# beast-dev/beast-mcmc

Measured on NVIDIA H100. Metric: tree log-likelihood evals/sec, higher is better.
Workload: dtype f64

## Files before the change

beast-mcmc_b200/csrc/api.cu:

```cuda
#include "../../include/libhmsbeagle_b200.h"
#include "engine.h"
#include "multi.h"

#include <algorithm>
#include <atomic>
#include <chrono>
#include <cmath>
#include <cstdio>
#include <cstdlib>
#include <cstring>
#include <string>
#include <unordered_map>

using namespace b200;

namespace {

std::mutex gMutex;
std::vector<Instance*> gInstances;

const long kSupportedFlags =
    BEAGLE_FLAG_PRECISION_DOUBLE | BEAGLE_FLAG_PRECISION_SINGLE | BEAGLE_FLAG_COMPUTATION_SYNCH | BEAGLE_FLAG_EIGEN_REAL |
    BEAGLE_FLAG_EIGEN_COMPLEX | BEAGLE_FLAG_SCALING_MANUAL | BEAGLE_FLAG_SCALING_DYNAMIC |
    BEAGLE_FLAG_SCALERS_RAW | BEAGLE_FLAG_SCALERS_LOG | BEAGLE_FLAG_VECTOR_NONE | BEAGLE_FLAG_THREADING_NONE |
// ... 58 lines not shown
            cudaEventCreate(&a);
            cudaEventCreate(&b);
            cudaEventRecord(a, in->stream);
        }
    }
    ~TimedScope() {
        if (in->timing) {
            cudaEventRecord(b, in->stream);
            in->timed[cls].push_back({a, b});
        }
    }
};

void* stage(Instance* in, const void* src, size_t bytes) {
    size_t need = (bytes + 255) & ~size_t(255);
    if (need > in->stageSize) return nullptr;
    if (in->stagePos + need > in->stageSize) {
        cudaStreamSynchronize(in->stream);
        in->stagePos = 0;
    }
    char* h = in->hStage + in->stagePos;
    char* d = in->dStage + in->stagePos;
    memcpy(h, src, bytes);
    if (cudaMemcpyAsync(d, h, bytes, cudaMemcpyHostToDevice, in->stream) != cudaSuccess) return nullptr;
    in->stagePos += need;
    return d;
}

int uploadSmall(Instance* in, void* dDst, const void* src, size_t bytes) {
    size_t need = (bytes + 255) & ~size_t(255);
    if (need > in->stageSize) return BEAGLE_ERROR_OUT_OF_RANGE;
    if (in->stagePos + need > in->stageSize) {
        cudaStreamSynchronize(in->stream);
        in->stagePos = 0;
    }
    char* h = in->hStage + in->stagePos;
    memcpy(h, src, bytes);
    in->stagePos += need;
    CUDA_OK(cudaMemcpyAsync(dDst, h, bytes, cudaMemcpyHostToDevice, in->stream));
    return BEAGLE_SUCCESS;
}

char* ensurePartials(Instance* in, int idx) {
    if (in->partials[idx] == nullptr) {
        if (in->nextSlot >= in->nSlots) return nullptr;
        in->slotOf[idx] = in->nextSlot++;
        in->partials[idx] = in->partialsBase + (size_t)in->slotOf[idx] * in->partialsElems * in->elemBytes();
    }
    return in->partials[idx];
}

bool validRange(int idx, int n) { return idx >= 0 && idx < n; }

void destroyInstance(Instance* in) {
    if (in->shard != nullptr) { shardedDestroy(in); delete in; return; }
    cudaSetDevice(in->device);
    exchangeRelease(in);
    if (in->stream) cudaStreamSynchronize(in->stream);
    cudaFree(in->partialsBase); cudaFree(in->states8Base); cudaFree(in->states32Base);
    for (CachedPlan& cp : in->planCache) { cp.dropGraph(); cudaFree(cp.dBlock); }
    cudaFree(in->dEigen); cudaFree(in->dMat); cudaFree(in->dEvec); cudaFree(in->dIncSums); cudaFree(in->dIncCounter);
    cudaFree(in->dRecipe);
    if (in->hMapped) cudaFreeHost(in->hMapped); cudaFree(in->dRates); cudaFree(in->dWeights);
    cudaFree(in->dFreqs); cudaFree(in->dScale); cudaFree(in->dPatternWeights);
    cudaFree(in->dPatternPartitions); cudaFree(in->dSite); cudaFree(in->dBlockSums); cudaFree(in->dOut);
    cudaFree(in->dCounter); cudaFree(in->dStage); cudaFree(in->dScratch);
    if (in->hStage) cudaFreeHost(in->hStage);
    if (in->hOut) cudaFreeHost(in->hOut);
    for (int c = 0; c < T_CLASSES; ++c)
        for (auto& ev : in->timed[c]) { cudaEventDestroy(ev.first); cudaEventDestroy(ev.second); }
    if (in->stream) cudaStreamDestroy(in->stream);
    delete in;
}

std::vector<BeagleResource> gResources;
std::vector<int> gShardDevices;
int gShardResource = -1;
std::vector<std::string> gResourceStrings;
BeagleResourceList gResourceList = {nullptr, 0};
std::once_flag gResourceOnce;

void buildResources() {
    int n = 0;
    if (cudaGetDeviceCount(&n) != cudaSuccess) { cudaGetLastError(); n = 0; }
    gResourceStrings.reserve(2 * (n + 1));
    gResourceStrings.push_back("CPU (host)");
    gResourceStrings.push_back("no host implementation in this library | use a GPU resource (1..N)");
    for (int d = 0; d < n; ++d) {
        cudaDeviceProp prop;
        if (cudaGetDeviceProperties(&prop, d) != cudaSuccess) { cudaGetLastError(); continue; }
        char buf[512];
        snprintf(buf, sizeof buf, "%s", prop.name);
        gResourceStrings.push_back(buf);
        snprintf(buf, sizeof buf, "Global memory (MB): %zu | SMs: %d | compute capability: %d.%d | "
                 "native walk kernels (sm_90a), fp64 arithmetic, fp64 or fp32 (4-state) partials",
                 (size_t)(prop.totalGlobalMem >> 20), prop.multiProcessorCount, prop.major, prop.minor);
        gResourceStrings.push_back(buf);
    }
    gShardDevices.clear();
    if (const char* env = getenv("B200_SHARD_DEVICES")) {
        for (const char* q = env; *q;) {
            char* end = nullptr;
            const long d = strtol(q, &end, 10);
            if (end == q) break;
            if (d >= 0 && d < n) gShardDevices.push_back((int)d);
            q = (*end == ',') ? end + 1 : end;
        }
    } else {
        for (int d = 0; d < n; ++d) gShardDevices.push_back(d);
    }
    if (gShardDevices.size() > (size_t)kMaxGroup) gShardDevices.resize(kMaxGroup);
    if (!gShardDevices.empty()) {
        char buf[512];
        snprintf(buf, sizeof buf, "GPU x %zu (pattern-sharded)", gShardDevices.size());
        gResourceStrings.push_back(buf);
        snprintf(buf, sizeof buf, "one instance over %zu GPUs | contiguous pattern blocks (Patterns.java:142-169 rule) | "
                 "per-shard sums added over NVLink inside the root kernel", gShardDevices.size());
        gResourceStrings.push_back(buf);
        gShardResource = (int)(gResourceStrings.size() / 2) - 1;
    }
    size_t count = gResourceStrings.size() / 2;
    gResources.resize(count);
    for (size_t r = 0; r < count; ++r) {
        gResources[r].name = const_cast<char*>(gResourceStrings[2 * r].c_str());
        gResources[r].description = const_cast<char*>(gResourceStrings[2 * r + 1].c_str());
        gResources[r].supportFlags = (r == 0) ? (BEAGLE_FLAG_PROCESSOR_CPU | BEAGLE_FLAG_FRAMEWORK_CPU) : kSupportedFlags;
        gResources[r].requiredFlags = (r == 0) ? BEAGLE_FLAG_FRAMEWORK_CPU : BEAGLE_FLAG_FRAMEWORK_CUDA;
    }
    gResourceList.list = gResources.data();
    gResourceList.length = (int)count;
}

char gImplName[] = "B200-CUDA-Double";
char gImplNameSingle[] = "B200-CUDA-Single";
char gImplDesc[] = "sm_90a walk kernels: one launch per operation list, shared-memory operand stack";


struct Sub { int begin, end, pBase, pLimit; };
struct Plan {
    std::vector<int> order;
    std::vector<Sub> subs;
    std::vector<int> phaseStart;
};

void planPhases(const std::vector<HostOp>& ops, int nBuffers, bool allowReorder, int fixedT, int wantSubs, int minT,
                int smallRemainder, Plan& plan) {
    const int n = (int)ops.size();
    auto single = [&]() {
        plan.order.resize(n);
        for (int k = 0; k < n; ++k) plan.order[k] = k;
        plan.subs.assign(1, Sub{0, n, 0, 0});
        plan.phaseStart = {0, 1};
    };
    if (!allowReorder || n < 2) { single(); return; }
    std::vector<int> writer(nBuffers, -1);
    for (int k = 0; k < n; ++k) {
        if (writer[ops[k].dest] >= 0) { single(); return; }
        writer[ops[k].dest] = k;
    }
    std::vector<int> ch0(n, -1), ch1(n, -1), parent(n, -1);
    for (int k = 0; k < n; ++k) {
        const int a = writer[ops[k].c1], b = writer[ops[k].c2];
        if (a >= 0) { if (a >= k || parent[a] >= 0) { single(); return; } ch0[k] = a; parent[a] = k; }
        if (b >= 0 && ops[k].c2 != ops[k].c1) { if (b >= k || parent[b] >= 0) { single(); return; } ch1[k] = b; parent[b] = k; }
        if (ops[k].dest == ops[k].c1 || ops[k].dest == ops[k].c2) { single(); return; }
    }
    std::vector<char> alive(n, 1);
    std::vector<int> size(n), need(n);
    std::vector<std::pair<int, int>> stack;
    plan.order.clear(); plan.order.reserve(n);
    plan.subs.clear(); plan.phaseStart.assign(1, 0);
    int remaining = n;
    while (remaining > 0) {
        const int T = fixedT > 0 ? fixedT : (remaining <= smallRemainder ? remaining : std::max(minT, (remaining + wantSubs - 1) / wantSubs));
        for (int k = 0; k < n; ++k) {
            if (!alive[k]) continue;
            const int a = (ch0[k] >= 0 && alive[ch0[k]]) ? ch0[k] : -1;
            const int b = (ch1[k] >= 0 && alive[ch1[k]]) ? ch1[k] : -1;
            size[k] = 1 + (a >= 0 ? size[a] : 0) + (b >= 0 ? size[b] : 0);
            int na = a >= 0 ? need[a] : 0, nb = b >= 0 ? need[b] : 0;
            if (na < nb) std::swap(na, nb);
            need[k] = std::max(1, std::max(na, nb + (nb > 0 ? 1 : 0)));
        }
        for (int r = 0; r < n; ++r) {
            if (!alive[r] || size[r] > T) continue;
            if (parent[r] >= 0 && size[parent[r]] <= T) continue;
            const int begin = (int)plan.order.size();
            stack.push_back({r, 0});
            while (!stack.empty()) {
                auto [k, stageNo] = stack.back();
                stack.pop_back();
                if (stageNo == 1) { plan.order.push_back(k); continue; }
                stack.push_back({k, 1});
                const int a = (ch0[k] >= 0 && alive[ch0[k]]) ? ch0[k] : -1;
                const int b = (ch1[k] >= 0 && alive[ch1[k]]) ? ch1[k] : -1;
                const int na = a >= 0 ? need[a] : -1, nb = b >= 0 ? need[b] : -1;
                if (na >= nb) { if (b >= 0) stack.push_back({b, 0}); if (a >= 0) stack.push_back({a, 0}); }
                else          { if (a >= 0) stack.push_back({a, 0}); if (b >= 0) stack.push_back({b, 0}); }
            }
            plan.subs.push_back(Sub{begin, (int)plan.order.size(), 0, 0});
        }
        for (int q = plan.subs[plan.phaseStart.back()].begin; q < (int)plan.order.size(); ++q) alive[plan.order[q]] = 0;
        std::stable_sort(plan.subs.begin() + plan.phaseStart.back(), plan.subs.end(),
                         [](const Sub& a, const Sub& b) { return (a.end - a.begin) > (b.end - b.begin); });
        remaining = n - (int)plan.order.size();
        plan.phaseStart.push_back((int)plan.subs.size());
    }
}

void planLevels(const std::vector<HostOp>& ops, int nBuffers, Plan& plan) {
    const int n = (int)ops.size();
    std::vector<int> writer(nBuffers, -1), level(n, 0);
    bool hazard = false;
    for (int k = 0; k < n; ++k) { if (writer[ops[k].dest] >= 0) hazard = true; writer[ops[k].dest] = k; }
    int maxLevel = 0;
    for (int k = 0; k < n && !hazard; ++k) {
        for (int src : {ops[k].c1, ops[k].c2}) {
            const int w = writer[src];
            if (w < 0) continue;
            if (w >= k) { hazard = true; break; }
            level[k] = std::max(level[k], level[w] + 1);
        }
        maxLevel = std::max(maxLevel, level[k]);
    }
    plan.order.resize(n);
    for (int k = 0; k < n; ++k) plan.order[k] = k;
    plan.subs.clear();
    if (hazard) { plan.subs.assign(1, Sub{0, n, 0, 0}); plan.phaseStart = {0, 1}; return; }
    std::stable_sort(plan.order.begin(), plan.order.end(), [&](int a, int b) { return level[a] < level[b]; });
    plan.phaseStart.assign(1, 0);
    for (int pos = 0; pos < n; ++pos) {
        if (pos > 0 && level[plan.order[pos]] != level[plan.order[pos - 1]]) plan.phaseStart.push_back((int)plan.subs.size());
        plan.subs.push_back(Sub{pos, pos + 1, 0, 0});
    }
    plan.phaseStart.push_back((int)plan.subs.size());
}

void planPreorderPhases(const std::vector<HostOp>& ops, int nBuffers, int fixedT, int wantSubs, int minT,
                        int smallRemainder, Plan& plan) {
    const int n = (int)ops.size();
    std::vector<int> writer(nBuffers, -1), parent(n, -1);
    bool ok = n >= 2;
    for (int k = 0; k < n && ok; ++k) { ok = writer[ops[k].dest] < 0; writer[ops[k].dest] = k; }
    for (int k = 0; k < n && ok; ++k) {
        const int a = writer[ops[k].c1];
        ok = writer[ops[k].c2] < 0 && (a < 0 || a < k) && ops[k].dest != ops[k].c1 && ops[k].dest != ops[k].c2;
        parent[k] = a;
    }
    if (!ok) { planLevels(ops, nBuffers, plan); return; }
    std::vector<std::vector<int>> kids(n);
    for (int k = 0; k < n; ++k) if (parent[k] >= 0) kids[parent[k]].push_back(k);
    std::vector<char> alive(n, 1);
    std::vector<int> size(n), stack;
    std::vector<std::vector<int>> phases;
    int remaining = n;
    while (remaining > 0) {
        const int T = fixedT > 0 ? fixedT : (remaining <= smallRemainder ? remaining : std::max(minT, (remaining + wantSubs - 1) / wantSubs));
        for (int k = n - 1; k >= 0; --k) {
            if (!alive[k]) continue;
            size[k] = 1;
            for (int c : kids[k]) if (alive[c]) size[k] += size[c];
        }
        std::vector<int> roots;
        for (int r = 0; r < n; ++r)
            if (alive[r] && size[r] <= T && !(parent[r] >= 0 && alive[parent[r]] && size[parent[r]] <= T)) roots.push_back(r);
        for (int r : roots) {
            stack.assign(1, r);
            while (!stack.empty()) {
                const int k = stack.back(); stack.pop_back();
                if (!alive[k]) continue;
                alive[k] = 0; --remaining;
                for (int c : kids[k]) if (alive[c]) stack.push_back(c);
            }
        }
        phases.push_back(std::move(roots));
    }
    std::vector<int> phaseOf(n, -1), rootOf(n, -1);
    for (int ph = 0; ph < (int)phases.size(); ++ph)
        for (int r : phases[ph]) { phaseOf[r] = ph; rootOf[r] = r; }
    for (int k = 0; k < n; ++k)
        if (rootOf[k] < 0) { rootOf[k] = rootOf[parent[k]]; phaseOf[k] = phaseOf[parent[k]]; }
    plan.order.clear(); plan.order.reserve(n);
    plan.subs.clear(); plan.phaseStart.assign(1, 0);
    for (int ph = (int)phases.size() - 1; ph >= 0; --ph) {
        for (int r : phases[ph]) {
            const int begin = (int)plan.order.size();
            stack.assign(1, r);
            while (!stack.empty()) {
                const int k = stack.back(); stack.pop_back();
                plan.order.push_back(k);
                for (int q = (int)kids[k].size() - 1; q >= 0; --q)
                    if (rootOf[kids[k][q]] == r) stack.push_back(kids[k][q]);
            }
            plan.subs.push_back(Sub{begin, (int)plan.order.size(), 0, 0});
        }
        std::stable_sort(plan.subs.begin() + plan.phaseStart.back(), plan.subs.end(),
                         [](const Sub& a, const Sub& b) { return (a.end - a.begin) > (b.end - b.begin); });
        plan.phaseStart.push_back((int)plan.subs.size());
    }
}

cudaError_t launchPlan(Instance* in, const void* dOps, const void* dSubs, const std::vector<int>& phaseStart,
                       const std::vector<int>& phaseDepth, bool fourPath, int maxWindow, bool preOrder, int eigenSlot = -1,
                       bool aligned = false, const void* dSnap = nullptr, int nSnap = 0, const void* dVirtTips = nullptr) {
    const bool virt = dVirtTips != nullptr;
    cudaError_t e = cudaSuccess;
    if (nSnap > 0) {
        TimedScope ts(in, T_PARTIALS);
        e = launchCherrySnapshot(in, static_cast<const int4*>(dSnap), nSnap);
    }
    for (size_t ph = 0; ph + 1 < phaseStart.size() && e == cudaSuccess; ++ph) {
        const int s0 = phaseStart[ph], s1 = phaseStart[ph + 1];
        if (s1 <= s0) continue;
        TimedScope ts(in, T_PARTIALS);
        if (fourPath && eigenSlot >= 0 && !preOrder && (ph >= phaseDepth.size() || phaseDepth[ph] == 0)) {
            e = launchWalk4E(in, static_cast<const Op4*>(dOps), static_cast<const int4*>(dSubs) + s0, s1 - s0, maxWindow,
                             aligned, in->hEigen.data() + (size_t)eigenSlot * 36, static_cast<const int4*>(dVirtTips));
            continue;
        }
        if (virt) return cudaErrorInvalidValue;
        e = fourPath ? launchWalk4(in, static_cast<const Op4*>(dOps), static_cast<const int4*>(dSubs) + s0, s1 - s0,
                                   ph < phaseDepth.size() ? phaseDepth[ph] : 0, maxWindow, preOrder)
                     : launchWalkGeneric(in, static_cast<const DevOp*>(dOps), static_cast<const int4*>(dSubs) + s0, s1 - s0,
                                         maxWindow, preOrder);
    }
    return e;
}

cudaError_t accumulateInList(Instance* in, const std::vector<CumGroup>& groups) {
    for (const CumGroup& g : groups) {
        int* dIdx = static_cast<int*>(stage(in, g.indices.data(), sizeof(int) * g.indices.size()));
        if (dIdx == nullptr) return cudaErrorMemoryAllocation;
        cudaError_t e = launchScaleAccumulate(in, dIdx, (int)g.indices.size(), in->dScale + (size_t)g.cum * in->Ppad, 1.0,
                                              g.pBegin, g.pEnd);
        if (e != cudaSuccess) return e;
        in->scaleIsLog[g.cum] = 1;
    }
    return cudaSuccess;
}

void noteScaleWrites(Instance* in, const std::vector<HostOp>& hops) {
    for (const HostOp& o : hops) if (o.sw >= 0) in->scaleIsLog[o.sw] = in->logScalers ? 1 : 0;
}


cudaError_t storeCherries(Instance* in, const int* bufs, int count) {
    if (in->cherryTip1.empty()) return cudaSuccess;
    std::vector<int4> items;
    for (int k = 0; k < count; ++k) {
        const int b = bufs[k];
        if (!validRange(b, in->nBuffers) || in->cherryTip1[b] < 0 || in->cherryStored[b]) continue;
        items.push_back(make_int4(in->slotOf[b], b, in->cherryTip1[b], in->cherryTip2[b]));
        in->cherryStored[b] = 1;
    }
    if (items.empty()) return cudaSuccess;
    const int4* dItems = static_cast<const int4*>(stage(in, items.data(), sizeof(int4) * items.size()));
    cudaError_t e = cudaErrorMemoryAllocation;
    if (dItems != nullptr) {
        TimedScope ts(in, T_PARTIALS);
        e = launchCherryStore(in, dItems, (int)items.size());
    }
    if (e != cudaSuccess) for (const int4& it : items) in->cherryStored[it.y] = 0;
    return e;
}

cudaError_t storeExternal(Instance* in, const std::vector<CherryRef>& external) {
    std::vector<int> bufs;
    for (const CherryRef& x : external) if (x.tip1 < 0) bufs.push_back(x.buf);
    return storeCherries(in, bufs.data(), (int)bufs.size());
}

cudaError_t settleCherriesOf(Instance* in, int t) {
    std::vector<int> deps;
    for (int b = 0; b < (int)in->cherryTip1.size(); ++b)
        if (in->cherryTip1[b] >= 0 && (in->cherryTip1[b] == t || in->cherryTip2[b] == t)) deps.push_back(b);
    const cudaError_t e = storeCherries(in, deps.data(), (int)deps.size());
    if (e == cudaSuccess) for (int b : deps) in->cherryTip1[b] = -1;
    return e;
}

void noteCherryWrites(Instance* in, const std::vector<HostOp>& hops, const std::vector<CherryRef>& cherries) {
    if (in->cherryTip1.empty()) return;
    for (const HostOp& o : hops) in->cherryTip1[o.dest] = -1;
    for (const CherryRef& c : cherries) {
        in->cherryTip1[c.buf] = c.tip1; in->cherryTip2[c.buf] = c.tip2; in->cherryStored[c.buf] = 0;
    }
}

int prepareOps(Instance* in, const std::vector<HostOp>& hops, bool byPartition) {
    for (const HostOp& o : hops) {
        if (!validRange(o.dest, in->nBuffers) || !validRange(o.c1, in->nBuffers) ||
            !validRange(o.c2, in->nBuffers) || !validRange(o.m1, in->nMatrices) ||
            !validRange(o.m2, in->nMatrices))
            return BEAGLE_ERROR_OUT_OF_RANGE;
        if (o.sw != BEAGLE_OP_NONE && !validRange(o.sw, in->nScale)) return BEAGLE_ERROR_OUT_OF_RANGE;
        if (o.sr != BEAGLE_OP_NONE && !validRange(o.sr, in->nScale)) return BEAGLE_ERROR_OUT_OF_RANGE;
        if (o.cum != BEAGLE_OP_NONE && !validRange(o.cum, in->nScale)) return BEAGLE_ERROR_OUT_OF_RANGE;
        if (byPartition && !validRange(o.part, in->partitionCount)) return BEAGLE_ERROR_OUT_OF_RANGE;
    }
    {
        std::vector<char> written(in->nBuffers, 0);
        for (const HostOp& o : hops) written[o.dest] = 1;
        auto holdsData = [&](int b) { return written[b] || in->partials[b] != nullptr || in->states32[b] != nullptr; };
        for (const HostOp& o : hops) {
            if (!holdsData(o.c1) || !holdsData(o.c2)) return BEAGLE_ERROR_OUT_OF_RANGE;
            if (o.kind == 1 && !written[o.c1] && in->states32[o.c1] != nullptr) return BEAGLE_ERROR_OUT_OF_RANGE;
        }
    }
    for (const HostOp& o : hops) {
        if (ensurePartials(in, o.dest) == nullptr) return BEAGLE_ERROR_OUT_OF_MEMORY;
        if (in->states32[o.dest] != nullptr) in->bufferEpoch++;
        in->states8[o.dest] = nullptr;
        in->states32[o.dest] = nullptr;
    }
    return BEAGLE_SUCCESS;
}

int eigenFormSlot(const Instance* in, const std::vector<HostOp>& hops) {
    if (!in->eigenWalk || in->matCP == 0 || in->walkVariant != 0 || hops.empty() || hops[0].kind == 1) return -1;
    const int E = in->matEigen[hops[0].m1];
    if (E < 0 || !in->eigenReal[E]) return -1;
    const unsigned gen = in->eigenGen[E];
    for (const HostOp& o : hops)
        if (in->matEigen[o.m1] != E || in->matEigen[o.m2] != E || in->matEigenGen[o.m1] != gen || in->matEigenGen[o.m2] != gen)
            return -1;
    return E;
}

int planAndLaunch(Instance* in, const std::vector<HostOp>& hops, bool byPartition) {
    const int n = (int)hops.size();
    if (n == 0) return BEAGLE_SUCCESS;
    static_assert(sizeof(HostOp) == 10 * sizeof(int), "HostOp is compared bytewise");
    if (in->planCacheSize > 0) {
        for (CachedPlan& cp : in->planCache) {
            if (cp.dBlock == nullptr || cp.n != n || cp.byPartition != byPartition || cp.epoch != in->bufferEpoch ||
                memcmp(cp.key.data(), hops.data(), sizeof(HostOp) * (size_t)n) != 0)
                continue;
            const int eigenSlot = cp.fourPath ? eigenFormSlot(in, hops) : -1;
            bool stale = cp.readsVirtual && eigenSlot < 0;
            for (const CherryRef& x : cp.external)
                stale = stale || (x.tip1 >= 0 && (in->cherryTip1[x.buf] != x.tip1 || in->cherryTip2[x.buf] != x.tip2));
            if (stale) { cp.dropGraph(); cp.n = -1; continue; }
            CUDA_OK(storeExternal(in, cp.external));
            cp.lastUse = ++in->planClock;
            cp.hits++;
            const unsigned eigenGenNow = eigenSlot >= 0 ? in->eigenGen[eigenSlot] : 0u;
            const void* dSnap = static_cast<char*>(cp.dBlock) + cp.snapOffset;
            const int nSnap = (int)cp.cherries.size();
            const void* dTips = cp.readsVirtual ? static_cast<char*>(cp.dBlock) + cp.tipsOffset : nullptr;
            if (cp.graphExec != nullptr && (cp.graphEigen != eigenSlot || cp.graphEigenGen != eigenGenNow)) {
                if (cp.graphAllEigen && eigenSlot >= 0 && cp.graphEigen == eigenSlot &&
                    updateWalk4EGraph(cp.graphExec, cp.graphKernelNodes, in->hEigen.data() + (size_t)eigenSlot * 36) == cudaSuccess) {
                    cp.graphEigenGen = eigenGenNow;
                } else {
                    cudaGetLastError();
                    cp.dropGraph();
                    cp.hits = 1;
                    if (++cp.graphInvalidations >= 4) cp.graphFailed = true;
                }
            }
            int launches = nSnap > 0;
            for (size_t ph = 0; ph + 1 < cp.phaseStart.size(); ++ph) launches += cp.phaseStart[ph + 1] > cp.phaseStart[ph];
            if (in->useGraphs && launches >= 2 && cp.cumGroups.empty()) {
                if (cp.graphExec == nullptr && !cp.graphFailed && cp.hits >= 2 && !in->timing &&
                    cudaStreamBeginCapture(in->stream, cudaStreamCaptureModeThreadLocal) == cudaSuccess) {
                    const cudaError_t e1 = launchPlan(in, cp.dBlock, static_cast<char*>(cp.dBlock) + cp.subsOffset, cp.phaseStart,
                                                      cp.phaseDepth, cp.fourPath, cp.maxWindow, cp.preOrder, eigenSlot,
                                                      !cp.byPartition, dSnap, nSnap, dTips);
                    cp.graphEigen = eigenSlot;
                    cp.graphEigenGen = eigenGenNow;
                    cudaGraph_t g = nullptr;
                    const cudaError_t e2 = cudaStreamEndCapture(in->stream, &g);
                    if (e1 != cudaSuccess || e2 != cudaSuccess || g == nullptr ||
                        cudaGraphInstantiate(&cp.graphExec, g, 0) != cudaSuccess) {
                        cp.graphExec = nullptr;
                        cp.graphFailed = true;
                        if (g) cudaGraphDestroy(g);
                    } else {
                        cp.graph = g;
                        cp.graphKernelNodes.clear();
                        cp.graphAllEigen = cp.fourPath && eigenSlot >= 0 && !cp.preOrder;
                        for (int dpt : cp.phaseDepth) cp.graphAllEigen = cp.graphAllEigen && dpt == 0;
                        size_t nn = 0;
                        if (cudaGraphGetNodes(g, nullptr, &nn) == cudaSuccess && nn > 0) {
                            std::vector<cudaGraphNode_t> nodes(nn);
                            cudaGraphNodeType ty;
                            if (cudaGraphGetNodes(g, nodes.data(), &nn) == cudaSuccess)
                                for (size_t q = 0; q < nn; ++q)
                                    if (cudaGraphNodeGetType(nodes[q], &ty) == cudaSuccess && ty == cudaGraphNodeTypeKernel)
                                        cp.graphKernelNodes.push_back(nodes[q]);
                        }
                        if (cp.graphKernelNodes.empty()) cp.graphAllEigen = false;
                    }
                    if (getenv("B200_BEAGLE_DEBUG"))
                        fprintf(stderr, "[b200-beagle] graph %s: %d launches\n", cp.graphExec ? "captured" : "capture failed",
                                launches);
                    cudaGetLastError();
                }
                if (cp.graphExec != nullptr) {
                    TimedScope ts(in, T_PARTIALS, launches);
                    CUDA_OK(cudaGraphLaunch(cp.graphExec, in->stream));
                    noteScaleWrites(in, hops);
                    noteCherryWrites(in, hops, cp.cherries);
                    return BEAGLE_SUCCESS;
                }
            }
            CUDA_OK(launchPlan(in, cp.dBlock, static_cast<char*>(cp.dBlock) + cp.subsOffset, cp.phaseStart, cp.phaseDepth,
                               cp.fourPath, cp.maxWindow, cp.preOrder, eigenSlot, !cp.byPartition, dSnap, nSnap,
                               dTips));
            CUDA_OK(accumulateInList(in, cp.cumGroups));
            noteScaleWrites(in, hops);
            noteCherryWrites(in, hops, cp.cherries);
            return BEAGLE_SUCCESS;
        }
    }
    {
        const int rcPrepare = prepareOps(in, hops, byPartition);
        if (rcPrepare != BEAGLE_SUCCESS) return rcPrepare;
    }
    const bool fourState = in->matCP > 0;
    const bool preOrder = hops[0].kind == 1;
    const int eigenSlot = fourState ? eigenFormSlot(in, hops) : -1;
    std::vector<char> written(in->nBuffers, 0);
    std::vector<int> firstWrite(in->nBuffers, n);
    for (int k = n - 1; k >= 0; --k) { written[hops[k].dest] = 1; firstWrite[hops[k].dest] = k; }
    std::vector<CherryRef> cherries;
    std::vector<int4> snap;
    std::vector<HostOp> kept;
    bool readsVirtual = false;
    if (!in->cherryTip1.empty() && !byPartition && !preOrder && eigenSlot >= 0 && !in->stackTail) {
        std::vector<int> writes(in->nBuffers, 0), firstRead(in->nBuffers, n);
        for (int k = 0; k < n; ++k) {
            writes[hops[k].dest]++;
            firstRead[hops[k].c1] = std::min(firstRead[hops[k].c1], k);
            firstRead[hops[k].c2] = std::min(firstRead[hops[k].c2], k);
        }
        for (int k = 0; k < n; ++k) {
            const HostOp& o = hops[k];
            if (in->states8[o.c1] != nullptr && in->states8[o.c2] != nullptr && o.sw == BEAGLE_OP_NONE &&
                o.sr == BEAGLE_OP_NONE && o.cum == BEAGLE_OP_NONE && writes[o.dest] == 1 && firstRead[o.dest] > k) {
                cherries.push_back(CherryRef{o.dest, o.c1, o.c2});
                snap.push_back(make_int4(o.dest, o.m1, o.m2, 0));
            } else {
                kept.push_back(o);
            }
        }
        if (kept.empty()) { cherries.clear(); snap.clear(); }
        readsVirtual = !cherries.empty();
        for (const HostOp& o : hops)
            for (int c : {o.c1, o.c2})
                readsVirtual = readsVirtual || (!written[c] && in->states32[c] == nullptr && in->cherryTip1[c] >= 0);
    }
    Plan plan;
    int maxWindow = in->Ppad;
    const int patsPerWarp = !fourState ? 16 : (in->walkVariant == 2 ? 8 * in->tensorR : (32 / in->matCP) * in->walkR);
    const int warpsPerSM = fourState ? 32 : 12;
    auto wantSubsFor = [&](int window) {
        const int warpsPerSub = std::max(1, (window + patsPerWarp - 1) / patsPerWarp);
        const int over = in->phaseOversub > 0 ? in->phaseOversub : (warpsPerSub >= 32 ? 1 : 2);
        return std::max(1, over * ((in->smCount * warpsPerSM + warpsPerSub - 1) / warpsPerSub));
    };
    if (!byPartition && !preOrder) {
        planPhases(cherries.empty() ? hops : kept, in->nBuffers, in->reorder != 0, in->phaseT, wantSubsFor(in->Ppad),
                   in->phaseTmin, in->phaseSmall, plan);
        bool served = true;
        for (size_t ph = 0; readsVirtual && ph + 1 < plan.phaseStart.size(); ++ph) {
            const int nSubs = plan.phaseStart[ph + 1] - plan.phaseStart[ph];
            served = served && (nSubs == 0 || walk4pServes(in, nSubs, in->Ppad));
        }
        if (!served) {
            readsVirtual = false;
            if (!cherries.empty()) {
                cherries.clear(); snap.clear(); kept.clear();
                planPhases(hops, in->nBuffers, in->reorder != 0, in->phaseT, wantSubsFor(in->Ppad), in->phaseTmin,
                           in->phaseSmall, plan);
            }
        }
        for (Sub& sb : plan.subs) { sb.pBase = 0; sb.pLimit = in->Ppad; }
    }
    const std::vector<HostOp>& L = cherries.empty() ? hops : kept;
    const int nL = (int)L.size();
    std::vector<int> vt1(readsVirtual ? in->nBuffers : 0, -1), vt2(readsVirtual ? in->nBuffers : 0, -1);
    for (const CherryRef& c : cherries) { vt1[c.buf] = c.tip1; vt2[c.buf] = c.tip2; }
    std::vector<CherryRef> external;
    {
        std::vector<char> seen(in->nBuffers, 0);
        for (int k = 0; k < n; ++k)
            for (int c : {hops[k].c1, hops[k].c2}) {
                if (firstWrite[c] < k || in->states32[c] != nullptr || seen[c]) continue;
                seen[c] = 1;
                const bool virt = readsVirtual && !written[c] && in->cherryTip1[c] >= 0;
                external.push_back(CherryRef{c, virt ? in->cherryTip1[c] : -1, virt ? in->cherryTip2[c] : -1});
                if (virt) { vt1[c] = in->cherryTip1[c]; vt2[c] = in->cherryTip2[c]; }
            }
    }
    CUDA_OK(storeExternal(in, external));
    {
        if (!byPartition) {
            if (preOrder) {
                if (in->prePhases) planPreorderPhases(hops, in->nBuffers, in->phaseT, wantSubsFor(in->Ppad), in->phaseTmin, in->phaseSmall, plan);
                else planLevels(hops, in->nBuffers, plan);
                for (Sub& sb : plan.subs) { sb.pBase = 0; sb.pLimit = in->Ppad; }
            }
        } else {
            std::vector<std::vector<int>> members(in->partitionCount);
            for (int k = 0; k < n; ++k) members[hops[k].part].push_back(k);
            std::vector<Plan> plans;
            std::vector<int> base;
            maxWindow = 1;
            for (int part = 0; part < in->partitionCount; ++part) {
                if (members[part].empty()) continue;
                std::vector<HostOp> sub(members[part].size());
                for (size_t q = 0; q < sub.size(); ++q) sub[q] = hops[members[part][q]];
                Plan pl;
                const int window = in->partEnd[part] - in->partBegin[part];
                if (sub[0].kind == 1 && in->prePhases) planPreorderPhases(sub, in->nBuffers, in->phaseT, wantSubsFor(std::max(1, window)), in->phaseTmin, in->phaseSmall, pl);
                else if (sub[0].kind == 1) planLevels(sub, in->nBuffers, pl);
                else planPhases(sub, in->nBuffers, in->reorder != 0, in->phaseT, wantSubsFor(std::max(1, window)), in->phaseTmin, in->phaseSmall, pl);
                base.push_back((int)plan.order.size());
                for (int idx : pl.order) plan.order.push_back(members[part][idx]);
                for (Sub& sb : pl.subs) {
                    sb.begin += base.back(); sb.end += base.back();
                    sb.pBase = in->partBegin[part]; sb.pLimit = in->partEnd[part];
                }
                maxWindow = std::max(maxWindow, window);
                plans.push_back(std::move(pl));
            }
            plan.phaseStart.assign(1, 0);
            for (size_t ph = 0;; ++ph) {
                bool any = false;
                for (const Plan& pl : plans) {
                    if (ph + 1 >= pl.phaseStart.size()) continue;
                    any = true;
                    for (int q = pl.phaseStart[ph]; q < pl.phaseStart[ph + 1]; ++q) plan.subs.push_back(pl.subs[q]);
                }
                if (!any) break;
                plan.phaseStart.push_back((int)plan.subs.size());
            }
        }
    }
    const std::vector<int>& order = plan.order;

    const bool stackEverywhere = fourState && in->walkVariant == 1 && !preOrder;
    const bool stackThin = fourState && in->walkVariant == 0 && in->stackTail && !preOrder;
    const int maxDepth = (stackEverywhere || stackThin) ? in->stackDepthMax : 0;
    const int nPhases = (int)plan.phaseStart.size() - 1;
    std::vector<char> subStack(plan.subs.size(), 0);
    std::vector<int> phaseDepth(std::max(nPhases, 1), 0), phaseOfSub(plan.subs.size(), 0);
    if (maxDepth > 0) {
        const int patsPerWarpS = (32 / in->matCP) * in->walkR;
        for (int ph = 0; ph < nPhases; ++ph) {
            long warps = 0;
            for (int q = plan.phaseStart[ph]; q < plan.phaseStart[ph + 1]; ++q) {
                warps += (plan.subs[q].pLimit - plan.subs[q].pBase + patsPerWarpS - 1) / patsPerWarpS;
                phaseOfSub[q] = ph;
            }
            const bool thin = warps < (long)in->smCount * 8;
            for (int q = plan.phaseStart[ph]; q < plan.phaseStart[ph + 1]; ++q) subStack[q] = stackEverywhere || thin;
        }
    }
    std::vector<int> lastReadOfProd(maxDepth > 0 ? nL : 0, -1);
    std::vector<int> subOfPos(nL, 0);
    for (int sIdx = 0; sIdx < (int)plan.subs.size(); ++sIdx)
        for (int q = plan.subs[sIdx].begin; q < plan.subs[sIdx].end; ++q) subOfPos[q] = sIdx;
    if (maxDepth > 0) {
        std::vector<int> lastRead(in->nBuffers, -1);
        for (size_t sIdx = 0; sIdx < plan.subs.size(); ++sIdx) {
            if (!subStack[sIdx]) continue;
            const Sub& sb = plan.subs[sIdx];
            for (int pos = sb.end - 1; pos >= sb.begin; --pos) {
                const HostOp& o = L[order[pos]];
                lastReadOfProd[pos] = lastRead[o.dest];
                lastRead[o.dest] = -1;
                if (lastRead[o.c1] < 0) lastRead[o.c1] = pos;
                if (lastRead[o.c2] < 0) lastRead[o.c2] = pos;
            }
            for (int pos = sb.begin; pos < sb.end; ++pos) {
                const HostOp& o = L[order[pos]];
                lastRead[o.dest] = lastRead[o.c1] = lastRead[o.c2] = -1;
            }
        }
    }
    std::vector<int> slotOf(maxDepth > 0 ? in->nBuffers : 0, -1), slotFreeAt(maxDepth > 0 ? in->nBuffers : 0, -1);
    std::vector<int> freeSlots;
    int depthUsed = 0, depthThisSub = 0, curSub = -1;

    const bool fourPath = in->matCP > 0;
    std::vector<CumGroup> cumGroups;
    std::vector<DevOp> dops(fourPath ? 0 : nL);
    std::vector<Op4> ops4(fourPath ? nL : 0);
    std::vector<int4> virtTips(readsVirtual ? nL : 0);
    for (int pos = 0; pos < nL; ++pos) {
        const HostOp& o = L[order[pos]];
        const bool t1 = in->states32[o.c1] != nullptr;
        const bool t2 = in->states32[o.c2] != nullptr;
        int srcSlot1 = -1, srcSlot2 = -1, dstSlot = -1;
        if (maxDepth > 0 && subOfPos[pos] != curSub) {
            curSub = subOfPos[pos];
            freeSlots.clear();
            depthThisSub = 0;
        }
        if (maxDepth > 0 && subStack[subOfPos[pos]]) {
            auto take = [&](int buf, bool isTip) -> int {
                if (isTip) return -1;
                const int slot = slotOf[buf];
                if (slot >= 0 && slotFreeAt[buf] == pos) { freeSlots.push_back(slot); slotOf[buf] = -1; }
                return slot;
            };
            srcSlot1 = take(o.c1, t1);
            srcSlot2 = (o.c2 == o.c1) ? srcSlot1 : take(o.c2, t2);
            if (slotOf[o.dest] >= 0) { freeSlots.push_back(slotOf[o.dest]); slotOf[o.dest] = -1; }
            if (lastReadOfProd[pos] > pos) {
                int slot = -1;
                if (!freeSlots.empty()) { slot = freeSlots.back(); freeSlots.pop_back(); }
                else if (depthThisSub < maxDepth) {
                    slot = depthThisSub++;
                    depthUsed = std::max(depthUsed, depthThisSub);
                    phaseDepth[phaseOfSub[subOfPos[pos]]] = std::max(phaseDepth[phaseOfSub[subOfPos[pos]]], depthThisSub);
                }
                if (slot >= 0) { slotOf[o.dest] = slot; slotFreeAt[o.dest] = lastReadOfProd[pos]; dstSlot = slot; }
            }
        }
        const int pBegin = byPartition ? in->partBegin[o.part] : 0;
        const int pEnd = byPartition ? in->partEnd[o.part] : in->P;
        if (o.cum >= 0 && o.sw >= 0) {
            CumGroup* grp = nullptr;
            for (CumGroup& g : cumGroups) if (g.cum == o.cum && g.pBegin == pBegin && g.pEnd == pEnd) { grp = &g; break; }
            if (grp == nullptr) { cumGroups.push_back(CumGroup{o.cum, pBegin, pEnd, {}}); grp = &cumGroups.back(); }
            grp->indices.push_back(o.sw);
        }
        const int cum = -1;
        if (fourPath) {
            Op4& d = ops4[pos];
            const bool v1 = readsVirtual && !t1 && vt1[o.c1] >= 0, v2 = readsVirtual && !t2 && vt1[o.c2] >= 0;
            d.dest = in->slotOf[o.dest];
            d.c1 = t1 ? -(o.c1 + 1) : v1 ? o.c1 : in->slotOf[o.c1];
            d.c2 = t2 ? -(o.c2 + 1) : v2 ? o.c2 : in->slotOf[o.c2];
            d.m1 = o.m1; d.m2 = o.m2; d.sw = o.sw; d.sr = o.sr; d.cum = cum;
            d.pBegin = pBegin; d.pEnd = pEnd;
            d.slots = (unsigned)(srcSlot1 & 0xFF) | ((unsigned)(srcSlot2 & 0xFF) << 8) | ((unsigned)(dstSlot & 0xFF) << 16);
            d.pad_ = o.kind | (v1 ? 4 : 0) | (v2 ? 8 : 0);
            d.pfA = d.pfB = 0; d.pfM1 = d.pfM2 = -1;
            if (readsVirtual)
                virtTips[pos] = make_int4(v1 ? vt1[o.c1] : 0, v1 ? vt2[o.c1] : 0, v2 ? vt1[o.c2] : 0, v2 ? vt2[o.c2] : 0);
            if (in->forward && !(maxDepth > 0 && subStack[subOfPos[pos]]) && pos > plan.subs[subOfPos[pos]].begin) {
                const Op4& pv = ops4[pos - 1];
                if (pv.pBegin == d.pBegin && pv.pEnd == d.pEnd) {
                    if (!t1 && !v1 && d.c1 == pv.dest) d.pad_ |= 2;
                    else if (!preOrder && !t2 && !v2 && d.c2 == pv.dest) {
                        std::swap(d.c1, d.c2); std::swap(d.m1, d.m2);
                        if (readsVirtual) { int4& t = virtTips[pos]; t = make_int4(t.z, t.w, t.x, t.y); }
                        d.pad_ = (d.pad_ & ~12) | (v1 ? 8 : 0) | 2;
                    }
                }
            }
        } else {
            DevOp& d = dops[pos];
            memset(&d, 0, sizeof d);
            d.dest = reinterpret_cast<double*>(in->partials[o.dest]);
            d.c1 = t1 ? nullptr : reinterpret_cast<const double*>(in->partials[o.c1]);
            d.c2 = t2 ? nullptr : reinterpret_cast<const double*>(in->partials[o.c2]);
            d.s1 = t1 ? (const void*)in->states32[o.c1] : nullptr;
            d.s2 = t2 ? (const void*)in->states32[o.c2] : nullptr;
            d.m1 = in->dMat + (size_t)o.m1 * in->matStride;
            d.m2 = in->dMat + (size_t)o.m2 * in->matStride;
            d.scaleWrite = o.sw >= 0 ? in->dScale + (size_t)o.sw * in->Ppad : nullptr;
            d.scaleRead = o.sr >= 0 ? in->dScale + (size_t)o.sr * in->Ppad : nullptr;
            d.cumScale = cum >= 0 ? in->dScale + (size_t)cum * in->Ppad : nullptr;
            d.pBegin = pBegin; d.pEnd = pEnd;
            d.srcSlot1 = d.srcSlot2 = d.dstSlot = -1;
            d.pad_ = o.kind;
            if (in->forward && !preOrder && pos > plan.subs[subOfPos[pos]].begin) {
                const DevOp& pv = dops[pos - 1];
                if (pv.pBegin == d.pBegin && pv.pEnd == d.pEnd) {
                    if (d.c1 != nullptr && d.c1 == pv.dest) d.pad_ |= 2;
                    else if (d.c2 != nullptr && d.c2 == pv.dest) {
                        std::swap(d.c1, d.c2); std::swap(d.s1, d.s2); std::swap(d.m1, d.m2); d.pad_ |= 2;
                    }
                }
            }
        }
    }
    if (fourPath && in->lookahead && (!preOrder || in->lookaheadPre)) {
        std::vector<char> thick(plan.subs.size(), 0);
        const long perSub = (maxWindow + (32 / in->matCP) * in->walkR - 1) / ((32 / in->matCP) * in->walkR);
        for (int ph = 0; ph < nPhases; ++ph) {
            const bool t = (long)(plan.phaseStart[ph + 1] - plan.phaseStart[ph]) * perSub >= (long)in->smCount * 8;
            for (int q = plan.phaseStart[ph]; q < plan.phaseStart[ph + 1]; ++q) thick[q] = t;
        }
        for (size_t sIdx = 0; sIdx < plan.subs.size(); ++sIdx) {
            if ((maxDepth > 0 && subStack[sIdx]) || (!thick[sIdx] && in->lookahead < 2)) continue;
            for (int pos = plan.subs[sIdx].begin; pos + 1 < plan.subs[sIdx].end; ++pos) {
                Op4& d = ops4[pos];
                const Op4& nx = ops4[pos + 1];
                auto enc = [&](int child, bool fromRegisters, bool virt) -> int {
                    if (fromRegisters || virt) return 0;
                    if (child < 0) return ((-child - 1) << 1) | 1;
                    return child == d.dest ? 0 : ((child + 1) << 1);
                };
                d.pfA = enc(nx.c1, (nx.pad_ & 2) != 0, (nx.pad_ & 4) != 0);
                d.pfB = enc(nx.c2, false, (nx.pad_ & 8) != 0);
                if (d.pfA == 0) { d.pfA = d.pfB; d.pfB = 0; }
                d.pfM1 = nx.m1; d.pfM2 = nx.m2;
            }
        }
    }
    if (fourPath && getenv("B200_BEAGLE_DEBUG")) {
        int fwd = 0, internal = 0;
        for (const Op4& d : ops4) { fwd += (d.pad_ & 2) != 0; internal += (d.c1 >= 0) + (d.c2 >= 0); }
        fprintf(stderr, "[b200-beagle] plan: %d ops (%zu virtual cherries), %zu subtrees, %d phases, %d internal children, "
                "%d forwarded in registers\n", nL, cherries.size(), plan.subs.size(), nPhases, internal, fwd);
    }
    const size_t opBytes = (fourPath ? sizeof(Op4) : sizeof(DevOp)) * (size_t)nL;
    const size_t subBytes = sizeof(Sub) * plan.subs.size();
    const size_t snapBytes = sizeof(int4) * snap.size();
    const size_t subsOffset = (opBytes + 255) & ~size_t(255);
    const size_t snapOffset = subsOffset + ((subBytes + 255) & ~size_t(255));
    const size_t tipsBytes = sizeof(int4) * virtTips.size();
    const size_t tipsOffset = snapOffset + ((snapBytes + 255) & ~size_t(255));
    const size_t blockBytes = tipsOffset + tipsBytes;
    std::vector<char> hBlock(blockBytes, 0);
    memcpy(hBlock.data(), fourPath ? (const void*)ops4.data() : (const void*)dops.data(), opBytes);
    memcpy(hBlock.data() + subsOffset, plan.subs.data(), subBytes);
    if (snapBytes) memcpy(hBlock.data() + snapOffset, snap.data(), snapBytes);
    if (tipsBytes) memcpy(hBlock.data() + tipsOffset, virtTips.data(), tipsBytes);
    void* dOps = stage(in, hBlock.data(), blockBytes);
    void* tmp = nullptr;
    if (dOps == nullptr) {
        CUDA_OK(cudaMalloc(&tmp, blockBytes));
        dOps = tmp;
        cudaError_t ce = cudaMemcpyAsync(dOps, hBlock.data(), blockBytes, cudaMemcpyHostToDevice, in->stream);
        if (ce == cudaSuccess) ce = cudaStreamSynchronize(in->stream);
        if (ce != cudaSuccess) { cudaFree(tmp); CUDA_OK(ce); }
    }
    void* dSubs = static_cast<char*>(dOps) + subsOffset;
    std::vector<int> depths(plan.phaseStart.size(), 0);
    for (size_t ph = 0; ph + 1 < plan.phaseStart.size(); ++ph) depths[ph] = (maxDepth > 0 && ph < phaseDepth.size()) ? phaseDepth[ph] : 0;
    cudaError_t e = launchPlan(in, dOps, dSubs, plan.phaseStart, depths, fourPath, maxWindow, preOrder, eigenSlot, !byPartition,
                               static_cast<char*>(dOps) + snapOffset, (int)snap.size(),
                               readsVirtual ? static_cast<char*>(dOps) + tipsOffset : nullptr);
    if (e == cudaSuccess) e = accumulateInList(in, cumGroups);
    noteScaleWrites(in, hops);
    if (e == cudaSuccess) noteCherryWrites(in, hops, cherries);
    if (e == cudaSuccess && tmp == nullptr && in->planCacheSize > 0) {
        if ((int)in->planCache.size() < in->planCacheSize) in->planCache.emplace_back();
        CachedPlan* slot = nullptr;
        for (CachedPlan& cp : in->planCache) {
            if (cp.dBlock == nullptr || cp.n < 0) { slot = &cp; break; }
            if (slot == nullptr || cp.lastUse < slot->lastUse) slot = &cp;
        }
        slot->dropGraph();
        slot->hits = 0;
        slot->graphFailed = false;
        slot->graphInvalidations = 0;
        if (slot->capacity < blockBytes) {
            if (slot->dBlock) cudaFree(slot->dBlock);
            slot->dBlock = nullptr; slot->capacity = 0;
            if (cudaMalloc(&slot->dBlock, blockBytes) == cudaSuccess) slot->capacity = blockBytes; else cudaGetLastError();
        }
        if (slot->dBlock != nullptr &&
            cudaMemcpyAsync(slot->dBlock, dOps, blockBytes, cudaMemcpyDeviceToDevice, in->stream) == cudaSuccess) {
            slot->key = hops; slot->n = n; slot->byPartition = byPartition; slot->epoch = in->bufferEpoch;
            slot->subsOffset = subsOffset; slot->snapOffset = snapOffset; slot->tipsOffset = tipsOffset;
            slot->cherries = cherries; slot->external = external; slot->readsVirtual = readsVirtual;
            slot->phaseStart = plan.phaseStart; slot->phaseDepth = depths;
            slot->fourPath = fourPath; slot->maxWindow = maxWindow; slot->preOrder = preOrder;
            slot->lastUse = ++in->planClock;
            slot->cumGroups = cumGroups;
            slot->graphFailed = !cumGroups.empty();
        } else if (slot->dBlock != nullptr) {
            slot->n = -1;
        }
    }
    if (tmp != nullptr) { cudaStreamSynchronize(in->stream); cudaFree(tmp); }
    CUDA_OK(e);
    return BEAGLE_SUCCESS;
}

}

namespace b200 {
Instance* instanceById(int id) { return getInstance(id); }
}

extern "C" {

#ifndef B200_SOURCE_HASH
#define B200_SOURCE_HASH "unhashed"
#endif
const char* beagleGetVersion(void) { return "4.0.1-b200+" B200_SOURCE_HASH; }
const char* b200GetSourceHash(void) { return B200_SOURCE_HASH; }

const char* beagleGetCitation(void) {
    return "H100-native tree-likelihood engine exposing the BEAGLE API.\n"
           "API after: Ayres et al. (2019) BEAGLE 3. Syst Biol 68:1052-1061.";
}

BeagleResourceList* beagleGetResourceList(void) {
    std::call_once(gResourceOnce, buildResources);
    return &gResourceList;
}

BeagleBenchmarkedResourceList* beagleGetBenchmarkedResourceList(
    int tipCount, int compactBufferCount, int stateCount, int patternCount, int categoryCount, int* resourceList,
    int resourceCount, long preferenceFlags, long requirementFlags, int eigenModelCount, int partitionCount,
    int calculateDerivatives, long benchmarkFlags);

int beagleCreateInstance(int tipCount, int partialsBufferCount, int compactBufferCount, int stateCount,
                         int patternCount, int eigenBufferCount, int matrixBufferCount, int categoryCount,
                         int scaleBufferCount, int* resourceList, int resourceCount, long preferenceFlags,
                         long requirementFlags, BeagleInstanceDetails* returnInfo) {
    if (tipCount < 0 || partialsBufferCount < 0 || compactBufferCount < 0 || stateCount < 2 ||
        patternCount < 1 || eigenBufferCount < 0 || matrixBufferCount < 0 || categoryCount < 1 ||
        scaleBufferCount < 0 || stateCount > 255)
        return BEAGLE_ERROR_OUT_OF_RANGE;
    if (requirementFlags & ~kSupportedFlags) return BEAGLE_ERROR_NO_RESOURCE;
    const bool singleFits = stateCount <= 4 && categoryCount <= 8;
    if (requirementFlags & BEAGLE_FLAG_PRECISION_SINGLE) {
        if (!singleFits || (requirementFlags & BEAGLE_FLAG_PRECISION_DOUBLE)) return BEAGLE_ERROR_NO_RESOURCE;
    }
    const bool single = singleFits && ((requirementFlags & BEAGLE_FLAG_PRECISION_SINGLE) ||
                                       ((preferenceFlags & BEAGLE_FLAG_PRECISION_SINGLE) &&
                                        !((preferenceFlags | requirementFlags) & BEAGLE_FLAG_PRECISION_DOUBLE)));
    BeagleResourceList* rl = beagleGetResourceList();
    int resource = -1;
    if (resourceList == nullptr || resourceCount <= 0) {
        if (rl->length > 1) resource = 1;
    } else {
        for (int k = 0; k < resourceCount; ++k)
            if (resourceList[k] >= 1 && resourceList[k] < rl->length) { resource = resourceList[k]; break; }
    }
    if (resource < 1) return BEAGLE_ERROR_NO_RESOURCE;

    if (resource == gShardResource) {
        Instance* parent = new Instance();
        parent->resource = resource;
        parent->device = gShardDevices[0];
        parent->P = patternCount; parent->S = stateCount; parent->C = categoryCount; parent->tipCount = tipCount;
        const int g = (int)gShardDevices.size();
        const int rc = shardedCreate(parent, g, gShardDevices.data(), tipCount, partialsBufferCount, compactBufferCount,
                                     stateCount, patternCount, eigenBufferCount, matrixBufferCount, categoryCount,
                                     scaleBufferCount, preferenceFlags, requirementFlags, returnInfo);
        if (rc != BEAGLE_SUCCESS) { delete parent; return rc; }
        if (returnInfo != nullptr) {
            returnInfo->resourceNumber = resource;
            returnInfo->resourceName = rl->list[resource].name;
            parent->flags = returnInfo->flags;
        }
        std::lock_guard<std::mutex> lock(gMutex);
        int id = -1;
        for (size_t k = 0; k < gInstances.size(); ++k) if (gInstances[k] == nullptr) { id = (int)k; break; }
        if (id < 0) { gInstances.push_back(nullptr); id = (int)gInstances.size() - 1; }
        gInstances[id] = parent;
        parent->id = id;
        return id;
    }

    Instance* in = new Instance();
    in->device = resource - 1;
    in->resource = resource;
    if (cudaSetDevice(in->device) != cudaSuccess) { delete in; return BEAGLE_ERROR_NO_RESOURCE; }
    in->tipCount = tipCount; in->nPartials = partialsBufferCount; in->nCompact = compactBufferCount;
    in->S = stateCount; in->P = patternCount; in->nEigen = eigenBufferCount; in->nMatrices = matrixBufferCount;
    in->C = categoryCount; in->nScale = scaleBufferCount;
    in->Sp = stateCount <= 4 ? 4 : ((stateCount + 7) / 8) * 8;
    in->Ppad = ((patternCount + 31) / 32) * 32;
    in->nBuffers = partialsBufferCount + compactBufferCount;
    in->nSets = std::max(1, eigenBufferCount);
    in->single = single;
    in->complexEigen = (requirementFlags | preferenceFlags) & BEAGLE_FLAG_EIGEN_COMPLEX;
    in->logScalers = (requirementFlags | preferenceFlags) & BEAGLE_FLAG_SCALERS_LOG;
    in->flags = (single ? BEAGLE_FLAG_PRECISION_SINGLE : BEAGLE_FLAG_PRECISION_DOUBLE) | BEAGLE_FLAG_COMPUTATION_SYNCH |
                BEAGLE_FLAG_SCALING_MANUAL |
                BEAGLE_FLAG_VECTOR_NONE | BEAGLE_FLAG_THREADING_NONE | BEAGLE_FLAG_PROCESSOR_GPU |
                BEAGLE_FLAG_FRAMEWORK_CUDA | BEAGLE_FLAG_PARALLELOPS_GRID |
                (in->complexEigen ? BEAGLE_FLAG_EIGEN_COMPLEX : BEAGLE_FLAG_EIGEN_REAL) |
                (in->logScalers ? BEAGLE_FLAG_SCALERS_LOG : BEAGLE_FLAG_SCALERS_RAW);
    if ((requirementFlags | preferenceFlags) & BEAGLE_FLAG_PREORDER_TRANSPOSE_AUTO) in->flags |= BEAGLE_FLAG_PREORDER_TRANSPOSE_AUTO;
    if ((requirementFlags | preferenceFlags) & BEAGLE_FLAG_SCALING_DYNAMIC) {
        in->flags &= ~BEAGLE_FLAG_SCALING_MANUAL;
        in->flags |= BEAGLE_FLAG_SCALING_DYNAMIC;
    }
    in->partialsElems = (size_t)in->C * in->Ppad * in->Sp;
    if (in->Sp == 4 && in->C <= 32) {
        int cp = 1;
        while (cp < in->C) cp <<= 1;
        in->matCP = cp;
        in->matStride = (size_t)16 * cp + 52 * (size_t)in->C;
        in->matStride = (in->matStride + 3) & ~size_t(3);
    } else {
        in->matCP = 0;
        in->matStride = (size_t)in->C * in->Sp * (in->Sp + 2 * (size_t)(in->Sp + 4));
    }
    in->slotOf.assign(in->nBuffers, -1);
    in->partials.assign(in->nBuffers, nullptr);
    in->states8.assign(in->nBuffers, nullptr);
    in->states32.assign(in->nBuffers, nullptr);
    in->scaleIsLog.assign(std::max(1, in->nScale), in->logScalers ? 1 : 0);
    in->matEigen.assign(std::max(1, in->nMatrices), -1);
    in->matEigenGen.assign(std::max(1, in->nMatrices), 0u);
    in->eigenGen.assign(std::max(1, in->nEigen), 0u);
    in->eigenReal.assign(std::max(1, in->nEigen), 0);
    in->hEigen.assign((size_t)std::max(1, in->nEigen) * 36, 0.0);
    in->eigenWalk = envInt("B200_EIGEN_WALK", 1);
    in->tipMode = envInt("B200_TIP_MODE", 3);
    in->thinTipMode = envInt("B200_THIN_TIP_MODE", in->tipMode);
    in->virtualCherries = envInt("B200_VIRTUAL_CHERRIES", 1);
    in->walkBlock = 128;
    in->walkVariant = envInt("B200_WALK_VARIANT", 0);
    in->reorder = envInt("B200_REORDER", 1);
    in->forward = envInt("B200_FORWARD", 1);
    in->lookahead = envInt("B200_LOOKAHEAD", 1);
    in->useGraphs = envInt("B200_GRAPHS", 1);
    in->prePhases = envInt("B200_PRE_PHASES", 1);
    in->lookaheadPre = envInt("B200_LOOKAHEAD_PRE", 1);
    in->planCacheSize = std::max(0, std::min(16, envInt("B200_PLAN_CACHE", 4)));
    in->planCache.reserve(16);
    in->thinR1 = envInt("B200_THIN_R1", 1);
    in->stackTail = envInt("B200_STACK_TAIL", 0);
    in->phaseT = envInt("B200_PHASE_T", 0);
    in->phaseTmin = std::max(1, envInt("B200_PHASE_TMIN", 4));
    in->phaseSmall = envInt("B200_PHASE_SMALL", 24);
    in->phaseOversub = std::max(0, envInt("B200_PHASE_OVERSUB", 0));
    in->walkMinBlocks = envInt("B200_WALK_MINB", 4);
    in->walkMinBlocksSet = getenv("B200_WALK_MINB") != nullptr;
    in->tensorR = envInt("B200_TENSOR_R", 2) >= 4 ? 4 : 2;
    in->genericMma = envInt("B200_GENERIC_MMA", 1);
    in->mmaWarps = envInt("B200_MMA_WARPS", 4) == 8 ? 8 : 4;
    cudaDeviceProp prop;
    bool ok = cudaGetDeviceProperties(&prop, in->device) == cudaSuccess;
    if (ok) { in->smCount = prop.multiProcessorCount; in->maxSmemOptin = prop.sharedMemPerBlockOptin; }
    in->walkR = envInt("B200_WALK_R", 4);
    if (in->walkR != 1 && in->walkR != 2 && in->walkR != 4 && in->walkR != 8) in->walkR = 4;
    if (getenv("B200_WALK_R") == nullptr && in->matCP > 0) {
        const int G = 32 / in->matCP;
        while (in->walkR > 1 && (in->Ppad + G * in->walkR - 1) / (G * in->walkR) < in->smCount) in->walkR >>= 1;
    }
    in->stackDepthMax = std::min(64, std::max(0, envInt("B200_STACK_DEPTH", 12)));
    if (single) { in->walkVariant = 0; in->stackTail = 0; }

    ok = ok && cudaStreamCreateWithFlags(&in->stream, cudaStreamNonBlocking) == cudaSuccess;
    const size_t eigenStride = 2 * (size_t)in->S * in->S + 2 * in->S;
    const size_t matElems = (size_t)in->nMatrices * in->matStride;
    const int rootBlocks = (in->Ppad + 255) / 256;
    in->stageSize = size_t(8) << 20;
    auto alloc = [&](auto** p, size_t elems) {
        if (!ok) return;
        using T = std::remove_pointer_t<std::remove_pointer_t<decltype(p)>>;
        size_t bytes = std::max<size_t>(elems, 1) * sizeof(T);
        ok = cudaMalloc(reinterpret_cast<void**>(p), bytes) == cudaSuccess &&
             cudaMemsetAsync(*p, 0, bytes, in->stream) == cudaSuccess;
    };
    alloc(&in->dEigen, std::max(1, in->nEigen) * eigenStride);
    alloc(&in->dMat, matElems);
    if (in->matCP > 0) alloc(&in->dEvec, (size_t)in->nMatrices * in->matCP * 4);
    if (in->matCP > 0 && in->matCP <= 8 && in->virtualCherries) {
        alloc(&in->dRecipe, (size_t)in->nBuffers * 32 * in->matCP);
        in->cherryTip1.assign(in->nBuffers, -1);
        in->cherryTip2.assign(in->nBuffers, -1);
        in->cherryStored.assign(in->nBuffers, 0);
    }
    if (in->matCP > 0 && in->matCP <= 8) {
        alloc(&in->dIncSums, (size_t)in->Ppad / 4 + 8);
        alloc(&in->dIncCounter, 4);
        in->fuseSmall = envInt("B200_FUSE", 1);
        if (ok && in->fuseSmall) {
            if (cudaHostAlloc(reinterpret_cast<void**>(&in->hMapped), 64, cudaHostAllocMapped) == cudaSuccess &&
                cudaHostGetDevicePointer(reinterpret_cast<void**>(&in->dMapped), in->hMapped, 0) == cudaSuccess) {
                memset(in->hMapped, 0, 64);
            } else {
                cudaGetLastError();
                if (in->hMapped) cudaFreeHost(in->hMapped);
                in->hMapped = nullptr;
            }
        }
    }
    alloc(&in->dRates, (size_t)in->nSets * in->C);
    alloc(&in->dWeights, (size_t)in->nSets * in->C);
    alloc(&in->dFreqs, (size_t)in->nSets * in->Sp);
    alloc(&in->dScale, (size_t)in->nScale * in->Ppad);
    alloc(&in->dPatternWeights, in->Ppad);
    alloc(&in->dPatternPartitions, in->Ppad);
    alloc(&in->dSite, in->Ppad);
    alloc(&in->dBlockSums, rootBlocks);
    alloc(&in->dOut, 1024);
    alloc(&in->dCounter, 4);
    alloc(&in->dStage, in->stageSize);
    alloc(&in->states8Base, (size_t)std::max(1, in->tipCount) * in->Ppad);
    alloc(&in->states32Base, (size_t)std::max(1, in->tipCount) * in->Ppad);
    if (ok) {
        int want[2] = {in->nPartials, std::max(1, in->nPartials - std::min(in->nCompact, in->tipCount))};
        for (int attempt = 0; attempt < 2 && in->partialsBase == nullptr; ++attempt) {
            size_t bytes = (size_t)want[attempt] * in->partialsElems * in->elemBytes();
            if (cudaMalloc(reinterpret_cast<void**>(&in->partialsBase), bytes) == cudaSuccess) in->nSlots = want[attempt];
            else { cudaGetLastError(); in->partialsBase = nullptr; }
        }
        if (in->partialsBase == nullptr) { destroyInstance(in); return BEAGLE_ERROR_OUT_OF_MEMORY; }
    }
    ok = ok && cudaMallocHost(reinterpret_cast<void**>(&in->hStage), in->stageSize) == cudaSuccess;
    ok = ok && cudaMallocHost(reinterpret_cast<void**>(&in->hOut), 1024 * sizeof(double)) == cudaSuccess;
    if (ok) {
        in->hRates.assign((size_t)in->nSets * in->C, 1.0);
        in->hWeights.assign((size_t)in->nSets * in->C, 0.0);
        in->hFreqs.assign((size_t)in->nSets * 4, 0.0);
        std::vector<double> ones((size_t)std::max(in->nSets * in->C, in->Ppad), 1.0);
        ok = cudaMemcpyAsync(in->dRates, ones.data(), sizeof(double) * in->nSets * in->C, cudaMemcpyHostToDevice,
                             in->stream) == cudaSuccess;
        std::vector<double> w(in->Ppad, 0.0);
        std::fill(w.begin(), w.begin() + in->P, 1.0);
        ok = ok && cudaMemcpyAsync(in->dPatternWeights, w.data(), sizeof(double) * in->Ppad, cudaMemcpyHostToDevice,
                                   in->stream) == cudaSuccess;
        ok = ok && cudaStreamSynchronize(in->stream) == cudaSuccess;
    }
    if (!ok) {
        cudaError_t e = cudaGetLastError();
        destroyInstance(in);
        return e == cudaErrorMemoryAllocation ? BEAGLE_ERROR_OUT_OF_MEMORY : BEAGLE_ERROR_GENERAL;
    }
    in->partitionCount = 1;
    in->partBegin.assign(1, 0);
    in->partEnd.assign(1, in->P);
    {
        std::lock_guard<std::mutex> lock(gMutex);
        int id = -1;
        for (size_t k = 0; k < gInstances.size(); ++k) if (gInstances[k] == nullptr) { id = (int)k; break; }
        if (id < 0) { gInstances.push_back(nullptr); id = (int)gInstances.size() - 1; }
        gInstances[id] = in;
        in->id = id;
    }
    if (returnInfo != nullptr) {
        returnInfo->resourceNumber = resource;
        returnInfo->resourceName = rl->list[resource].name;
        returnInfo->implName = single ? gImplNameSingle : gImplName;
        returnInfo->implDescription = gImplDesc;
        returnInfo->flags = in->flags;
    }
    return in->id;
}

int beagleFinalizeInstance(int instance) {
    Instance* in = nullptr;
    {
        std::lock_guard<std::mutex> lock(gMutex);
        if (instance < 0 || instance >= (int)gInstances.size() || gInstances[instance] == nullptr)
            return BEAGLE_ERROR_UNINITIALIZED_INSTANCE;
        in = gInstances[instance];
        gInstances[instance] = nullptr;
    }
    destroyInstance(in);
    return BEAGLE_SUCCESS;
}

int beagleFinalize(void) {
    std::vector<Instance*> all;
    {
        std::lock_guard<std::mutex> lock(gMutex);
        all.swap(gInstances);
    }
    for (Instance* in : all) if (in) destroyInstance(in);
    return BEAGLE_SUCCESS;
}

int beagleSetCPUThreadCount(int instance, int) {
    SH(instance, BEAGLE_SUCCESS);
    GET_INSTANCE(in, instance);
    (void)in;
    return BEAGLE_SUCCESS;
}

int beagleSetTipStates(int instance, int tipIndex, const int* inStates) {
    SH(instance, shSetTipStates(sh, tipIndex, inStates));
    GET_INSTANCE(in, instance);
    if (!validRange(tipIndex, in->nBuffers) || inStates == nullptr) return BEAGLE_ERROR_OUT_OF_RANGE;
    std::vector<int> s32(in->Ppad, in->S);
    std::vector<uint8_t> s8(in->Ppad, (uint8_t)in->S);
    for (int p = 0; p < in->P; ++p) {
        int s = inStates[p];
        if (s < 0 || s >= in->S) s = in->S;
        s32[p] = s;
        s8[p] = (uint8_t)s;
    }
    if (tipIndex >= in->tipCount) return BEAGLE_ERROR_OUT_OF_RANGE;
    CUDA_OK(settleCherriesOf(in, tipIndex));
    in->states32[tipIndex] = in->states32Base + (size_t)tipIndex * in->Ppad;
    in->states8[tipIndex] = in->states8Base + (size_t)tipIndex * in->Ppad;
    CUDA_OK(cudaMemcpyAsync(in->states32[tipIndex], s32.data(), sizeof(int) * in->Ppad, cudaMemcpyHostToDevice, in->stream));
    CUDA_OK(cudaMemcpyAsync(in->states8[tipIndex], s8.data(), in->Ppad, cudaMemcpyHostToDevice, in->stream));
    CUDA_OK(cudaStreamSynchronize(in->stream));
    in->bufferEpoch++;
    return BEAGLE_SUCCESS;
}

int beagleGetTipStates(int instance, int tipIndex, int* outStates) {
    SH(instance, shGetTipStates(sh, tipIndex, outStates));
    GET_INSTANCE(in, instance);
    if (!validRange(tipIndex, in->nBuffers) || in->states32[tipIndex] == nullptr) return BEAGLE_ERROR_OUT_OF_RANGE;
    CUDA_OK(cudaMemcpyAsync(outStates, in->states32[tipIndex], sizeof(int) * in->P, cudaMemcpyDeviceToHost, in->stream));
    CUDA_OK(cudaStreamSynchronize(in->stream));
    return BEAGLE_SUCCESS;
}

static int setPartialsImpl(Instance* in, int bufferIndex, const double* inPartials, bool perCategory) {
    if (!validRange(bufferIndex, in->nBuffers) || inPartials == nullptr) return BEAGLE_ERROR_OUT_OF_RANGE;
    char* dst = ensurePartials(in, bufferIndex);
    if (dst == nullptr) return BEAGLE_ERROR_OUT_OF_MEMORY;
    CUDA_OK(settleCherriesOf(in, bufferIndex));
    if (!in->cherryTip1.empty()) in->cherryTip1[bufferIndex] = -1;
    std::vector<double> tmp(in->partialsElems, 0.0);
    for (int c = 0; c < in->C; ++c)
        for (int p = 0; p < in->Ppad; ++p) {
            double* row = tmp.data() + ((size_t)c * in->Ppad + p) * in->Sp;
            if (p < in->P) {
                const double* src = inPartials + ((size_t)(perCategory ? c : 0) * in->P + p) * in->S;
                for (int i = 0; i < in->S; ++i) row[i] = src[i];
            } else {
                for (int i = 0; i < in->S; ++i) row[i] = 1.0;
            }
        }
    if (in->single) {
        std::vector<float> narrow(in->partialsElems);
        for (size_t q = 0; q < narrow.size(); ++q) {
            const float f = (float)tmp[q];
            narrow[q] = std::fpclassify(f) == FP_SUBNORMAL ? std::copysign(0.0f, f) : f;
        }
        CUDA_OK(cudaMemcpyAsync(dst, narrow.data(), sizeof(float) * narrow.size(), cudaMemcpyHostToDevice, in->stream));
        CUDA_OK(cudaStreamSynchronize(in->stream));
    } else {
        CUDA_OK(cudaMemcpyAsync(dst, tmp.data(), sizeof(double) * in->partialsElems, cudaMemcpyHostToDevice, in->stream));
        CUDA_OK(cudaStreamSynchronize(in->stream));
    }
    if (in->states32[bufferIndex] != nullptr) in->bufferEpoch++;
    in->states32[bufferIndex] = nullptr;
    in->states8[bufferIndex] = nullptr;
    return BEAGLE_SUCCESS;
}

int beagleSetTipPartials(int instance, int tipIndex, const double* inPartials) {
    SH(instance, shSetPartials(sh, tipIndex, inPartials, false));
    GET_INSTANCE(in, instance);
    return setPartialsImpl(in, tipIndex, inPartials, false);
}

int beagleSetPartials(int instance, int bufferIndex, const double* inPartials) {
    SH(instance, shSetPartials(sh, bufferIndex, inPartials, true));
    GET_INSTANCE(in, instance);
    return setPartialsImpl(in, bufferIndex, inPartials, true);
}

int beagleGetPartials(int instance, int bufferIndex, int scaleIndex, double* outPartials) {
    SH(instance, shGetPartials(sh, bufferIndex, scaleIndex, outPartials));
    GET_INSTANCE(in, instance);
    if (!validRange(bufferIndex, in->nBuffers) || in->partials[bufferIndex] == nullptr || outPartials == nullptr)
        return BEAGLE_ERROR_OUT_OF_RANGE;
    if (scaleIndex != BEAGLE_OP_NONE && !validRange(scaleIndex, in->nScale)) return BEAGLE_ERROR_OUT_OF_RANGE;
    CUDA_OK(storeCherries(in, &bufferIndex, 1));
    std::vector<double> tmp(in->partialsElems);
    const double* src = reinterpret_cast<const double*>(in->partials[bufferIndex]);
    double* dTmp = nullptr;
    if (in->single) {
        std::vector<float> narrow(in->partialsElems);
        CUDA_OK(cudaMemcpyAsync(narrow.data(), in->partials[bufferIndex], sizeof(float) * narrow.size(),
                                cudaMemcpyDeviceToHost, in->stream));
        CUDA_OK(cudaStreamSynchronize(in->stream));
        for (size_t q = 0; q < narrow.size(); ++q) tmp[q] = narrow[q];
    }
    if (scaleIndex != BEAGLE_OP_NONE) {
        CUDA_OK(cudaMalloc(reinterpret_cast<void**>(&dTmp), sizeof(double) * in->partialsElems));
        if (in->single) {
            const cudaError_t eUp = cudaMemcpyAsync(dTmp, tmp.data(), sizeof(double) * in->partialsElems,
                                                    cudaMemcpyHostToDevice, in->stream);
            if (eUp != cudaSuccess) { cudaFree(dTmp); CUDA_OK(eUp); }
        } else {
            CUDA_OK(cudaMemcpyAsync(dTmp, src, sizeof(double) * in->partialsElems, cudaMemcpyDeviceToDevice, in->stream));
        }
        CUDA_OK(launchRescalePartialsForGet(in, dTmp, in->dScale + (size_t)scaleIndex * in->Ppad));
        src = dTmp;
    }
    cudaError_t e = cudaSuccess;
    if (!in->single || dTmp != nullptr) {
        e = cudaMemcpyAsync(tmp.data(), src, sizeof(double) * in->partialsElems, cudaMemcpyDeviceToHost, in->stream);
        if (e == cudaSuccess) e = cudaStreamSynchronize(in->stream);
    }
    if (dTmp) cudaFree(dTmp);
    CUDA_OK(e);
    for (int c = 0; c < in->C; ++c)
        for (int p = 0; p < in->P; ++p)
            memcpy(outPartials + ((size_t)c * in->P + p) * in->S, tmp.data() + ((size_t)c * in->Ppad + p) * in->Sp,
                   sizeof(double) * in->S);
    return BEAGLE_SUCCESS;
}

int beagleSetEigenDecomposition(int instance, int eigenIndex, const double* inEigenVectors,
                                const double* inInverseEigenVectors, const double* inEigenValues) {
    SH(instance, shBroadcast(sh, [&](int c) { return beagleSetEigenDecomposition(c, eigenIndex, inEigenVectors, inInverseEigenVectors, inEigenValues); }));
    GET_INSTANCE(in, instance);
    if (!validRange(eigenIndex, in->nEigen)) return BEAGLE_ERROR_OUT_OF_RANGE;
    const size_t S = in->S, stride = 2 * S * S + 2 * S;
    std::vector<double> pack(stride, 0.0);
    memcpy(pack.data(), inEigenVectors, sizeof(double) * S * S);
    memcpy(pack.data() + S * S, inInverseEigenVectors, sizeof(double) * S * S);
    memcpy(pack.data() + 2 * S * S, inEigenValues, sizeof(double) * (in->complexEigen ? 2 * S : S));
    if (in->matCP > 0) {
        double h[36] = {0.0};
        for (size_t k = 0; k < S; ++k) h[32 + k] = inEigenValues[k];
        for (size_t i = 0; i < S; ++i)
            for (size_t k = 0; k < S; ++k) { h[4 * i + k] = inEigenVectors[i * S + k]; h[16 + 4 * i + k] = inInverseEigenVectors[i * S + k]; }
        bool real = true;
        if (in->complexEigen) for (size_t k = 0; k < S; ++k) real = real && inEigenValues[S + k] == 0.0;
        double* dst = in->hEigen.data() + (size_t)eigenIndex * 36;
        if (memcmp(dst, h, sizeof h) != 0 || in->eigenGen[eigenIndex] == 0 || (bool)in->eigenReal[eigenIndex] != real) {
            memcpy(dst, h, sizeof h);
            in->eigenGen[eigenIndex]++;
        }
        in->eigenReal[eigenIndex] = real ? 1 : 0;
    }
    return uploadSmall(in, in->dEigen + (size_t)eigenIndex * stride, pack.data(), sizeof(double) * stride);
}

int beagleSetStateFrequencies(int instance, int stateFrequenciesIndex, const double* inStateFrequencies) {
    SH(instance, shBroadcast(sh, [&](int c) { return beagleSetStateFrequencies(c, stateFrequenciesIndex, inStateFrequencies); }));
    GET_INSTANCE(in, instance);
    if (!validRange(stateFrequenciesIndex, in->nSets)) return BEAGLE_ERROR_OUT_OF_RANGE;
    std::vector<double> f(in->Sp, 0.0);
    memcpy(f.data(), inStateFrequencies, sizeof(double) * in->S);
    if (in->hFreqs.size() == (size_t)in->nSets * 4 && in->S <= 4)
        for (int i = 0; i < 4; ++i) in->hFreqs[(size_t)stateFrequenciesIndex * 4 + i] = i < in->S ? inStateFrequencies[i] : 0.0;
    return uploadSmall(in, in->dFreqs + (size_t)stateFrequenciesIndex * in->Sp, f.data(), sizeof(double) * in->Sp);
}

int beagleSetCategoryWeights(int instance, int categoryWeightsIndex, const double* inCategoryWeights) {
    SH(instance, shBroadcast(sh, [&](int c) { return beagleSetCategoryWeights(c, categoryWeightsIndex, inCategoryWeights); }));
    GET_INSTANCE(in, instance);
    if (!validRange(categoryWeightsIndex, in->nSets)) return BEAGLE_ERROR_OUT_OF_RANGE;
    std::copy(inCategoryWeights, inCategoryWeights + in->C, in->hWeights.begin() + (size_t)categoryWeightsIndex * in->C);
    return uploadSmall(in, in->dWeights + (size_t)categoryWeightsIndex * in->C, inCategoryWeights, sizeof(double) * in->C);
}

int beagleSetCategoryRatesWithIndex(int instance, int categoryRatesIndex, const double* inCategoryRates) {
    SH(instance, shBroadcast(sh, [&](int c) { return beagleSetCategoryRatesWithIndex(c, categoryRatesIndex, inCategoryRates); }));
    GET_INSTANCE(in, instance);
    if (!validRange(categoryRatesIndex, in->nSets)) return BEAGLE_ERROR_OUT_OF_RANGE;
    std::copy(inCategoryRates, inCategoryRates + in->C, in->hRates.begin() + (size_t)categoryRatesIndex * in->C);
    return uploadSmall(in, in->dRates + (size_t)categoryRatesIndex * in->C, inCategoryRates, sizeof(double) * in->C);
}

int beagleSetCategoryRates(int instance, const double* inCategoryRates) {
    return beagleSetCategoryRatesWithIndex(instance, 0, inCategoryRates);
}

int beagleSetPatternWeights(int instance, const double* inPatternWeights) {
    SH(instance, shSetPatternWeights(sh, inPatternWeights));
    GET_INSTANCE(in, instance);
    std::vector<double> w(in->Ppad, 0.0);
    memcpy(w.data(), inPatternWeights, sizeof(double) * in->P);
    CUDA_OK(cudaMemcpyAsync(in->dPatternWeights, w.data(), sizeof(double) * in->Ppad, cudaMemcpyHostToDevice, in->stream));
    CUDA_OK(cudaStreamSynchronize(in->stream));
    return BEAGLE_SUCCESS;
}

int beagleSetPatternPartitions(int instance, int partitionCount, const int* inPatternPartitions) {
    SH(instance, BEAGLE_ERROR_NO_IMPLEMENTATION);
    GET_INSTANCE(in, instance);
// ... 913 lines not shown
```

beast-mcmc_b200/csrc/engine.h:

```cpp
#pragma once
#include <cuda_runtime.h>
#include <cstdint>
#include <mutex>
#include <vector>

namespace b200 {

struct alignas(16) DevOp {
    double* dest;
    const double* c1;
    const double* c2;
    const void* s1;
    const void* s2;
    const double* m1;
    const double* m2;
    double* scaleWrite;
    const double* scaleRead;
    double* cumScale;
    int pBegin, pEnd;
    int srcSlot1, srcSlot2;
    int dstSlot;
    int pad_;
};

struct alignas(16) Op4 {
    int dest, c1, c2, m1;
    int m2, sw, sr, cum;
    int pBegin, pEnd;
    unsigned int slots;
    int pad_;
    int pfA, pfB, pfM1, pfM2;
};

struct CherryRef { int buf, tip1, tip2; };

template <typename T> struct EdgeRefT { const T* post; const int* states; const T* pre; const double* D; double len; };
using EdgeRef = EdgeRefT<double>;

struct HostOp { int dest, sw, sr, c1, m1, c2, m2, part, cum; int kind = 0; };
struct CumGroup { int cum, pBegin, pEnd; std::vector<int> indices; };
struct CachedPlan {
    std::vector<HostOp> key;
    std::vector<CumGroup> cumGroups;
    int n = -1;
    bool byPartition = false, fourPath = false, preOrder = false;
    unsigned long epoch = 0;
    void* dBlock = nullptr;
    size_t capacity = 0, subsOffset = 0, snapOffset = 0, tipsOffset = 0;
    std::vector<CherryRef> cherries, external;
    bool readsVirtual = false;
    std::vector<int> phaseStart, phaseDepth;
    int maxWindow = 0;
    long lastUse = 0;
    long hits = 0;
    cudaGraphExec_t graphExec = nullptr;
    bool graphFailed = false;
    int graphEigen = -2;
    unsigned graphEigenGen = 0;
    int graphInvalidations = 0;
    cudaGraph_t graph = nullptr;
    std::vector<cudaGraphNode_t> graphKernelNodes;
    bool graphAllEigen = false;
    void dropGraph() {
        if (graphExec) cudaGraphExecDestroy(graphExec);
        if (graph) cudaGraphDestroy(graph);
        graphExec = nullptr; graph = nullptr; graphKernelNodes.clear(); graphAllEigen = false;
    }
};

enum TimingClass { T_PARTIALS = 0, T_MATRICES = 1, T_ROOT = 2, T_CLASSES = 3 };

constexpr int kIncMaxOps = 64, kIncMaxMats = 8;
struct IncOp { int dest, c1, c2, m1, m2, sw, sr, flags; };
struct IncMat { int prob, rateSet; double len; };
struct IncArgs {
    void* partials; size_t stride; const uint8_t* states; double* mats; double* evecs; double* scale;
    size_t matStride;
    int S, C, Ppad, P, logScalers, nOps, nMats, pad_;
    double V[16], Vi[16], eval[4];
    double weights[8], freqs[4], rate[kIncMaxMats][8];
    const double* cum; const double* patternWeights;
    double* site; double* blockSums; unsigned int* counter; double* out;
    volatile double* hostOut; volatile unsigned long long* hostFlag; unsigned long long seq;
    IncMat mat[kIncMaxMats];
    IncOp op[kIncMaxOps];
};

constexpr int kMaxGroup = 16;
struct ExchangeSlot { double value; unsigned long long seq; };
struct Exchange {
    int rank = 0, size = 1;
    unsigned long long seq = 0;
    long long timeoutCycles = 0;
    ExchangeSlot* peers[kMaxGroup] = {};
};

struct Instance {
    int id = -1, device = 0, resource = 0;
    int tipCount = 0, nPartials = 0, nCompact = 0, S = 0, P = 0, nEigen = 0, nMatrices = 0, C = 0, nScale = 0;
    int Sp = 0, Ppad = 0, nBuffers = 0, nSets = 1;
    long flags = 0;
    bool logScalers = false, complexEigen = false;
    cudaStream_t stream = nullptr;
    int smCount = 132;
    size_t maxSmemOptin = 0;

    bool single = false;
    size_t partialsElems = 0;
    size_t elemBytes() const { return single ? sizeof(float) : sizeof(double); }
    char* partialsBase = nullptr;
    int nSlots = 0, nextSlot = 0;
    std::vector<int> slotOf;
    std::vector<char*> partials;
    uint8_t* states8Base = nullptr;
    int* states32Base = nullptr;
    std::vector<uint8_t*> states8;
    std::vector<int*> states32;
    int matCP = 0;
    size_t matStride = 0;

    double* dEigen = nullptr;
    double* dMat = nullptr;
    double* dEvec = nullptr;
    std::vector<int> matEigen;
    std::vector<unsigned> matEigenGen, eigenGen;
    std::vector<char> eigenReal;
    std::vector<double> hEigen;
    int eigenWalk = 1;
    int tipMode = 2;
    int thinTipMode = 3;
    int virtualCherries = 1;
    std::vector<int> cherryTip1, cherryTip2;
    std::vector<char> cherryStored;
    double* dRecipe = nullptr;
    double* dRates = nullptr;
    std::vector<double> hRates, hWeights, hFreqs;
    double* dWeights = nullptr;
    double* dFreqs = nullptr;
    double* dScale = nullptr;
    std::vector<char> scaleIsLog;
    double* dPatternWeights = nullptr;
    int* dPatternPartitions = nullptr;
    double* dSite = nullptr;
    double* dBlockSums = nullptr;
    double* dOut = nullptr;
    unsigned int* dCounter = nullptr;
    int lookaheadPre = 1;
    int prePhases = 1;
    int useGraphs = 1;
    int lookahead = 1;
    int forward = 1;
    double* dScratch = nullptr;
    size_t scratchDoubles = 0;
    int partitionCount = 1;
    std::vector<int> partBegin, partEnd;
    std::vector<int> hostPartitions;

    char* hStage = nullptr;
    char* dStage = nullptr;
    size_t stageSize = 0, stagePos = 0;
    double* hOut = nullptr;

    int fuseSmall = 1;
    struct PendingMat { int prob, eigen, rateSet; double len; };
    std::vector<PendingMat> pendingMats;
    std::vector<HostOp> pendingOps;
    int pendingCum = -1;
    double* hMapped = nullptr;
    double* dMapped = nullptr;
    double* dIncSums = nullptr;
    unsigned int* dIncCounter = nullptr;
    unsigned long long incSeq = 0;
    long fusedLaunches = 0;

    void* shard = nullptr;
    Exchange exchange;
    ExchangeSlot* dSlots = nullptr;
    std::vector<void*> ipcOpened;
    bool exchangeOn = false;

    bool timing = false;
    std::vector<std::pair<cudaEvent_t, cudaEvent_t>> timed[T_CLASSES];
    double timedMs[T_CLASSES] = {0, 0, 0};
    long timedLaunches[T_CLASSES] = {0, 0, 0};

    size_t walkSmemConfigured = 0, genericSmemConfigured = 0, mmaSmemConfigured[8] = {0, 0, 0, 0, 0, 0, 0, 0};
    int walkBlock = 128;
    int walkVariant = 0;
    std::vector<CachedPlan> planCache;
    int planCacheSize = 4;
    long planClock = 0;
    unsigned long bufferEpoch = 0;
    int reorder = 1;
    int thinR1 = 1;
    int stackTail = 0;
    int stackDepthMax = 12;
    int walkMinBlocks = 4;
    bool walkMinBlocksSet = false;
    int mmaWarps = 4;
    int tensorR = 2;
    int genericMma = 1;
    int walkR = 4;
    int phaseTmin = 4, phaseOversub = 0, phaseSmall = 24;
    int phaseT = 0;
};

struct Sharded;
Instance* instanceById(int id);
void exchangeRelease(Instance* in);
int shardedCreate(Instance* parent, int g, const int* devices, int tipCount, int partialsBufferCount, int compactBufferCount,
                  int stateCount, int patternCount, int eigenBufferCount, int matrixBufferCount, int categoryCount,
                  int scaleBufferCount, long preferenceFlags, long requirementFlags, void* details );
void shardedDestroy(Instance* parent);

cudaError_t launchTransitionMatrices(Instance* in, const int* dProbIdx, const int* dEigenIdx,
                                     const int* dRateSet, const double* dLengths, int count);
cudaError_t launchWalk4(Instance* in, const Op4* dOps, const int4* dSubs, int nSubs, int stackDepth, int maxWindow, bool preOrder);
cudaError_t updateWalk4EGraph(cudaGraphExec_t exec, const std::vector<cudaGraphNode_t>& kernelNodes, const double* eigen);
cudaError_t launchWalk4E(Instance* in, const Op4* dOps, const int4* dSubs, int nSubs, int maxWindow, bool aligned,
                         const double* eigen, const int4* dVirtTips);
bool walk4pServes(const Instance* in, int nSubs, int maxWindow);
cudaError_t launchCherrySnapshot(Instance* in, const int4* dItems, int count);
cudaError_t launchCherryStore(Instance* in, const int4* dItems, int count);
cudaError_t launchWalkGeneric(Instance* in, const DevOp* dOps, const int4* dSubs, int nSubs, int maxWindow, bool preOrder);
size_t edgeDerivativeWorkspace(const Instance* in, int count);
cudaError_t launchEdgeDerivatives(Instance* in, const EdgeRefT<void>* dEdges, int count, const double* weights, double* outPerPattern,
                                  double* outSum, double* outSumSq, double* partial);
int compressSitePatterns(int device, int taxa, int sites, const int* hStates, int* hPatternOfSite, int* hPatterns,
                         double* hWeights, int* hPatternCount);
int crossProductBlocks(const Instance* in, int count);
cudaError_t launchCrossProducts(Instance* in, const EdgeRefT<void>* dEdges, int count, const double* rates,
                                const double* weights, double* scratch);
cudaError_t launchRoot(Instance* in, const void* root, const double* weights, const double* freqs,
                       const double* cumScale, int pBegin, int pEnd, double* dOutSlot, const Exchange* exchange = nullptr);
cudaError_t launchIncremental(Instance* in, const IncArgs& args);
cudaError_t launchCombineMatrices(Instance* in, const int* dFirst, const int* dSecond, const int* dResult, int count, bool multiply);
cudaError_t launchExchangeSum(Instance* in, const double* dVals, int n, double* dOutJoint, const Exchange* exchange);
cudaError_t launchScaleAccumulate(Instance* in, const int* dIdx, int count, double* cum, double sign,
                                  int pBegin, int pEnd);
cudaError_t launchRescalePartialsForGet(Instance* in, double* tmp, const double* cum);

}
```

beast-mcmc_b200/csrc/walk4e.cu:

```cuda
#include "engine.h"
#include "walk4.cuh"

namespace b200 {

namespace {

__device__ __forceinline__ double absBits(double v) {
    return __hiloint2double(__double2hiint(v) & 0x7fffffff, __double2loint(v));
}

template <typename T, int CP, int R, bool ALIGNED, bool FIRST, int TIP>
__device__ __forceinline__ void childTermE(const WalkArgs& A, const double (&Vi)[16], int child, int matIdx, bool fromRegisters,
                                           int cc, size_t off0, int p0, bool catValid, int pBegin, int pEnd, double (&d)[R][4],
                                           double* tab) {
    constexpr int G = 32 / CP;
    const int S = A.S;
    const bool tip = child < 0;
    if (TIP == 2 && tip) {
        const int lane = threadIdx.x & 31;
        const uint8_t* t = A.states + (size_t)(-child - 1) * A.Ppad;
        int s[R];
#pragma unroll
        for (int r = 0; r < R; ++r) {
            const int p = p0 + r * G;
            s[r] = (ALIGNED || (catValid && p >= pBegin && p < pEnd)) ? (int)__ldg(t + p) : 4;
        }
        const double* m = A.mats + (size_t)matIdx * A.matStride;
        __syncwarp();
#pragma unroll
        for (int q = lane; q < 5 * CP; q += 32) {
            const int c = q / 5, sym = q - 5 * c;
            double v[4];
            if (sym < S && sym < 4 && c < A.C) ldg256_ro(m + (sym * CP + c) * 4, v);
            else {
#pragma unroll
                for (int i = 0; i < 4; ++i) v[i] = (i < S) ? 1.0 : 0.0;
            }
            double2* dst = reinterpret_cast<double2*>(tab + q * 4);
            dst[0] = make_double2(v[0], v[1]);
            dst[1] = make_double2(v[2], v[3]);
        }
        __syncwarp();
#pragma unroll
        for (int r = 0; r < R; ++r) {
            const double2* col = reinterpret_cast<const double2*>(tab + (cc * 5 + min(s[r], 4)) * 4);
            const double2 lo = col[0], hi = col[1];
            if (FIRST) { d[r][0] = lo.x; d[r][1] = lo.y; d[r][2] = hi.x; d[r][3] = hi.y; }
            else { d[r][0] *= lo.x; d[r][1] *= lo.y; d[r][2] *= hi.x; d[r][3] *= hi.y; }
        }
        return;
    }
    if (TIP == 1 && tip) {
        const uint8_t* t = A.states + (size_t)(-child - 1) * A.Ppad;
        const double* m = A.mats + (size_t)matIdx * A.matStride + cc * 4;
#pragma unroll
        for (int r = 0; r < R; ++r) {
            const int p = p0 + r * G;
            const int s = (ALIGNED || (catValid && p >= pBegin && p < pEnd)) ? (int)__ldg(t + p) : S;
            double v[4];
            if (s < S) ldg256_ro(m + 4 * CP * s, v);
            else {
#pragma unroll
                for (int i = 0; i < 4; ++i) v[i] = (i < S) ? 1.0 : 0.0;
            }
#pragma unroll
            for (int i = 0; i < 4; ++i) d[r][i] = FIRST ? v[i] : d[r][i] * v[i];
        }
        return;
    }
    double e[4];
    ldg256_ro(A.evecs + ((size_t)matIdx * CP + cc) * 4, e);
    const uint8_t* t = A.states + (size_t)(tip ? -child - 1 : 0) * A.Ppad;
    const T* xg = static_cast<const T*>(A.partials) + (size_t)(tip ? 0 : child) * A.stride + off0;
#pragma unroll
    for (int r = 0; r < R; ++r) {
        const int p = p0 + r * G;
        const bool live = ALIGNED || (catValid && p >= pBegin && p < pEnd);
        double x[4], u[4], y[4];
        int s = 0;
        if (tip) {
            s = live ? (int)__ldg(t + p) : S;
#pragma unroll
            for (int j = 0; j < 4; ++j) x[j] = (s == j) ? 1.0 : 0.0;
        } else if (fromRegisters) {
#pragma unroll
            for (int i = 0; i < 4; ++i) x[i] = d[r][i];
        } else if (live) {
            loadCell(xg + (size_t)r * G * 4, x);
        } else {
            x[0] = x[1] = x[2] = x[3] = 0.0;
        }
#pragma unroll
        for (int k = 0; k < 4; ++k)
            u[k] = (Vi[4 * k] * x[0] + Vi[4 * k + 1] * x[1] + Vi[4 * k + 2] * x[2] + Vi[4 * k + 3] * x[3]) * e[k];
#pragma unroll
        for (int i = 0; i < 4; ++i)
            y[i] = absBits(A.V[4 * i] * u[0] + A.V[4 * i + 1] * u[1] + A.V[4 * i + 2] * u[2] + A.V[4 * i + 3] * u[3]);
        if (tip && s >= S) {
#pragma unroll
            for (int i = 0; i < 4; ++i) y[i] = (i < S) ? 1.0 : 0.0;
        }
#pragma unroll
        for (int i = 0; i < 4; ++i) d[r][i] = FIRST ? y[i] : d[r][i] * y[i];
    }
}

template <typename T, int CP, int R, bool ALIGNED, int TIP>
__device__ __forceinline__ void walk4eBody(const WalkArgs& A) {
    constexpr int G = 32 / CP;
    const int lane = threadIdx.x & 31;
    const int warp = (blockIdx.x * blockDim.x + threadIdx.x) >> 5;
    const int c = lane / G;
    const int4 range = __ldg(A.subs + blockIdx.y);
    const int p0 = range.z + warp * (G * R) + (lane % G);
    if (range.z + warp * (G * R) >= range.w) return;
    const bool catValid = c < A.C;
    const int cc = catValid ? c : 0;
    const size_t off0 = ((size_t)cc * A.Ppad + p0) * 4;
    const int last = range.y - 1;
    __shared__ __align__(16) double tipTab[TIP == 2 ? 4 * 2 * CP * 20 : 2];
    double* tab1 = tipTab + (TIP == 2 ? ((threadIdx.x >> 5) * 2) * CP * 20 : 0);
    double* tab2 = tab1 + (TIP == 2 ? CP * 20 : 0);

    double Vi[16];
#pragma unroll
    for (int q = 0; q < 16; ++q) asm volatile("mov.f64 %0, %1;" : "=d"(Vi[q]) : "d"(A.Vi[q]));
    Op4 cur = loadOp(A.ops + range.x);
    double d[R][4];
#pragma unroll
    for (int r = 0; r < R; ++r) d[r][0] = d[r][1] = d[r][2] = d[r][3] = 0.0;
    for (int k = range.x; k <= last; ++k) {
        Op4 nxt;
        if (R == 1) nxt = loadOp(A.ops + min(k + 1, last));
        else if (lane == 0) prefetchL1(A.ops + min(k + 2, last));
#pragma unroll
        for (int w = 0; w < 2; ++w) {
            const int pf = w == 0 ? cur.pfA : cur.pfB;
            if (pf == 0) continue;
            if (pf & 1) {
                const uint8_t* t = A.states + (size_t)(pf >> 1) * A.Ppad + p0;
                if ((lane % G) == 0 && c == 0) prefetchL1(t);
            } else if (catValid) {
                const T* xg = static_cast<const T*>(A.partials) + (size_t)((pf >> 1) - 1) * A.stride + off0;
#pragma unroll
                for (int r = 0; r < R; ++r)
                    if (ALIGNED || p0 + r * G < A.Ppad) prefetchL1(xg + (size_t)r * G * 4);
            }
        }
        if (lane < 2) {
            const int mi = lane == 0 ? cur.pfM1 : cur.pfM2;
            if (mi >= 0) prefetchL1(A.evecs + (size_t)mi * CP * 4);
        } else if (TIP != 0 && lane >= 8 && lane < 16) {
            const int mi = lane < 12 ? cur.pfM1 : cur.pfM2;
            if (mi >= 0) prefetchL1(A.mats + (size_t)mi * A.matStride + (lane & 3) * 4 * CP);
        }
        childTermE<T, CP, R, ALIGNED, true, TIP>(A, Vi, cur.c1, cur.m1, (cur.pad_ & 2) != 0, cc, off0, p0, catValid, cur.pBegin, cur.pEnd, d, tab1);
        childTermE<T, CP, R, ALIGNED, false, TIP>(A, Vi, cur.c2, cur.m2, false, cc, off0, p0, catValid, cur.pBegin, cur.pEnd, d, tab2);
        if (R != 1) nxt = loadOp(A.ops + min(k + 1, last));
        T* dg = static_cast<T*>(A.partials) + (size_t)cur.dest * A.stride + off0;
#pragma unroll
        for (int r = 0; r < R; ++r) {
            const int p = p0 + r * G;
            const bool active = ALIGNED ? catValid : (catValid && p >= cur.pBegin && p < cur.pEnd);
            if (cur.sw >= 0) {
                double m = active ? fmax(fmax(d[r][0], d[r][1]), fmax(d[r][2], d[r][3])) : 0.0;
#pragma unroll
                for (int sh = G; sh < 32; sh <<= 1) m = fmax(m, __shfl_xor_sync(0xffffffffu, m, sh));
                if (m == 0.0) m = 1.0;
                const double inv = 1.0 / m;
#pragma unroll
                for (int i = 0; i < 4; ++i) d[r][i] *= inv;
                if (active && c == 0) A.scale[(size_t)cur.sw * A.Ppad + p] = A.logScalers ? log(m) : m;
            } else if (cur.sr >= 0) {
                double f = active ? A.scale[(size_t)cur.sr * A.Ppad + p] : 1.0;
                if (A.logScalers) f = exp(f);
                const double inv = 1.0 / f;
#pragma unroll
                for (int i = 0; i < 4; ++i) d[r][i] *= inv;
            }
            roundCell<T>(d[r]);
            if (active) storeCell(dg + (size_t)r * G * 4, d[r]);
        }
        cur = nxt;
    }
}

template <int CP, int R, bool ALIGNED, int MINB, int TIP>
__global__ void __launch_bounds__(128, MINB)
k_walk4e(const WalkArgs A) {
    walk4eBody<double, CP, R, ALIGNED, TIP>(A);
}

template <int CP, int R, bool ALIGNED, int MINB, int TIP>
__global__ void __launch_bounds__(128, MINB)
k_walk4es(const WalkArgs A) {
    walk4eBody<float, CP, R, ALIGNED, TIP>(A);
}

__device__ __forceinline__ void cpAsync16(void* smemDst, const void* gmemSrc) {
    const unsigned sAddr = (unsigned)__cvta_generic_to_shared(smemDst);
    asm volatile("cp.async.ca.shared.global [%0], [%1], 16;" :: "r"(sAddr), "l"(gmemSrc) : "memory");
}
template <int BYTES>
__device__ __forceinline__ void cpAsyncSmall(void* smemDst, const void* gmemSrc) {
    const unsigned sAddr = (unsigned)__cvta_generic_to_shared(smemDst);
    asm volatile("cp.async.ca.shared.global [%0], [%1], %2;" :: "r"(sAddr), "l"(gmemSrc), "n"(BYTES) : "memory");
}

template <int CP, int R, bool VIRT>
struct WarpStage {
    static constexpr int G = 32 / CP, NP = G * R, TABLES = VIRT ? 4 : 2;
    double mat[TABLES][5 * CP * 4];
    double ev[2][CP * 4];
    alignas(16) unsigned char st[TABLES][NP < 16 ? 16 : NP];
};

template <typename T, int CP, int R, bool VIRT>
__device__ __forceinline__ void walk4pBody(const WalkArgs& A) {
    constexpr int G = 32 / CP, NP = G * R;
    constexpr int PIECE = NP < 16 ? NP : 16;
    static_assert(NP % PIECE == 0 && (PIECE == 4 || PIECE == 8 || PIECE == 16), "state-byte staging");
    constexpr int TABLES = WarpStage<CP, R, VIRT>::TABLES;
    constexpr int RECQ = sizeof(Op4) / 16 + (VIRT ? 1 : 0);
    __shared__ __align__(16) WarpStage<CP, R, VIRT> stages[4][2];
    __shared__ __align__(16) Op4 rings[4][4];
    __shared__ __align__(16) int4 tipRings[4][VIRT ? 4 : 1];
    int lane;
    asm volatile("mov.u32 %0, %%laneid;" : "=r"(lane));
    const int wib = threadIdx.x >> 5;
    const int warp = (blockIdx.x * blockDim.x + threadIdx.x) >> 5;
    const int c = lane / G;
    const int4 range = __ldg(A.subs + blockIdx.y);
    const int pBase = range.z + warp * NP;
    if (pBase >= range.w) return;
    const int p0 = pBase + (lane % G);
    const bool catValid = c < A.C;
    const int cc = catValid ? c : 0;
    const size_t off0 = ((size_t)cc * A.Ppad + p0) * 4;
    const int last = range.y - 1, S = A.S;
    WarpStage<CP, R, VIRT>* stage = stages[wib];
    Op4* ring = rings[wib];
    int4* tipRing = tipRings[wib];

    for (int q = lane; q < 2 * TABLES * CP * 4; q += 32) {
        const int tbl = q / (CP * 4), e = q % (CP * 4), gc = e >> 2, i = e & 3;
        stage[tbl / TABLES].mat[tbl % TABLES][(i >> 1) * 10 * CP + 2 * (4 * CP + gc) + (i & 1)] = (i < S) ? 1.0 : 0.0;
    }
    auto stageBlock = [&](double* tab, const double* src) {
#pragma unroll
        for (int q = lane; q < CP * 8; q += 32)
            cpAsync16(&tab[(q & 1) * 10 * CP + 2 * (((q >> 1) % CP) * 4 + q / (2 * CP))], src + 2 * q);
    };
    auto fetchRecord = [&](int j) {
        if (VIRT && lane == RECQ - 1) cpAsync16(&tipRing[j & 3], A.virtTips + j);
        else cpAsync16(reinterpret_cast<char*>(&ring[j & 3]) + 16 * lane, reinterpret_cast<const char*>(A.ops + j) + 16 * lane);
    };
    struct Rec { int dest, c1, c2, sw, sr, flags, pfA, pfB; };
    auto issueOperands = [&](int j) -> Rec {
        const int4 rec = *reinterpret_cast<const int4*>(&ring[j & 3]);
        const int4 rec2 = *(reinterpret_cast<const int4*>(&ring[j & 3]) + 1);
        const int flags = ring[j & 3].pad_;
        const int2 pf = *reinterpret_cast<const int2*>(&ring[j & 3].pfA);
        const int m2 = rec2.x;
        WarpStage<CP, R, VIRT>& sg = stage[j & 1];
#pragma unroll
        for (int ch = 0; ch < 2; ++ch) {
            const int child = ch == 0 ? rec.y : rec.z, m = ch == 0 ? rec.w : m2;
            const bool virt = VIRT && (flags & (4 << ch)) != 0;
            if (child < 0) {
                stageBlock(sg.mat[ch], A.mats + (size_t)m * A.matStride);
            } else {
                if (virt) {
                    const double* rcp = A.recipes + (size_t)child * 32 * CP;
                    stageBlock(sg.mat[ch], rcp);
                    stageBlock(sg.mat[TABLES - 2 + ch], rcp + 16 * CP);
                }
                if (lane < CP * 2) cpAsync16(&sg.ev[ch][2 * lane], A.evecs + (size_t)m * CP * 4 + 2 * lane);
            }
        }
        constexpr int SL = NP / PIECE;
        auto statePiece = [&](int q) {
            const int t = q / SL, piece = q % SL, ch = t & 1;
            const int child = ch == 0 ? rec.y : rec.z;
            int tip = t < 2 && child < 0 ? -child - 1 : -1;
            if (VIRT && (flags & (4 << ch)) != 0) {
                const int4 vt = tipRing[j & 3];
                tip = t == 0 ? vt.x : t == 1 ? vt.z : t == 2 ? vt.y : vt.w;
            }
            if (tip >= 0) cpAsyncSmall<PIECE>(&sg.st[t][PIECE * piece], A.states + (size_t)tip * A.Ppad + pBase + PIECE * piece);
        };
        if (lane < RECQ) {
            if (j + 1 <= last) fetchRecord(j + 1);
        } else if (lane < RECQ + TABLES * SL) {
            statePiece(lane - RECQ);
        }
        if constexpr (RECQ + TABLES * SL > 32) {
            if (lane < RECQ + TABLES * SL - 32) statePiece(lane + 32 - RECQ);
        }
        asm volatile("cp.async.commit_group;" ::: "memory");
        return Rec{rec.x, rec.y, rec.z, rec2.y, rec2.z, flags, pf.x, pf.y};
    };
    if (lane < RECQ) fetchRecord(range.x);
    asm volatile("cp.async.commit_group;" ::: "memory");
    asm volatile("cp.async.wait_group 0;" ::: "memory");
    __syncwarp();
    Rec nxt = issueOperands(range.x);
    asm volatile("cp.async.wait_group 0;" ::: "memory");
    __syncwarp();

    double Vi[16];
#pragma unroll
    for (int q = 0; q < 16; ++q) asm volatile("mov.f64 %0, %1;" : "=d"(Vi[q]) : "d"(A.Vi[q]));
    double d[R][4];
#pragma unroll
    for (int r = 0; r < R; ++r) d[r][0] = d[r][1] = d[r][2] = d[r][3] = 0.0;

    for (int k = range.x; k <= last; ++k) {
        const Rec cur = nxt;
        if (k + 1 <= last) nxt = issueOperands(k + 1);
        const WarpStage<CP, R, VIRT>& sg = stage[k & 1];
#pragma unroll
        for (int w = 0; w < 2; ++w) {
            const int pf = w == 0 ? cur.pfA : cur.pfB;
            if (pf == 0 || (pf & 1) || !catValid) continue;
            const T* xg = static_cast<const T*>(A.partials) + (size_t)((pf >> 1) - 1) * A.stride + off0;
#pragma unroll
            for (int r = 0; r < R; ++r) prefetchL1(xg + (size_t)r * G * 4);
        }
#pragma unroll
        for (int ch = 0; ch < 2; ++ch) {
            const int child = ch == 0 ? cur.c1 : cur.c2;
            if (child < 0) {
#pragma unroll
                for (int r = 0; r < R; ++r) {
                    const int sym = sg.st[ch][(lane % G) + r * G];
                    const int e2 = 2 * (sym < S ? cc * 4 + sym : 4 * CP + cc);
                    const double2 lo = *reinterpret_cast<const double2*>(&sg.mat[ch][e2]);
                    const double2 hi = *reinterpret_cast<const double2*>(&sg.mat[ch][10 * CP + e2]);
                    if (ch == 0) { d[r][0] = lo.x; d[r][1] = lo.y; d[r][2] = hi.x; d[r][3] = hi.y; }
                    else { d[r][0] *= lo.x; d[r][1] *= lo.y; d[r][2] *= hi.x; d[r][3] *= hi.y; }
                }
            } else {
                const double2* ep = reinterpret_cast<const double2*>(&sg.ev[ch][cc * 4]);
                const double2 e01 = ep[0], e23 = ep[1];
                const double e[4] = {e01.x, e01.y, e23.x, e23.y};
                const bool fromRegisters = ch == 0 && (cur.flags & 2) != 0;
                const bool virt = VIRT && (cur.flags & (4 << ch)) != 0;
                const T* xg = static_cast<const T*>(A.partials) + (size_t)child * A.stride + off0;
#pragma unroll
                for (int r = 0; r < R; ++r) {
                    double x[4], u[4], y[4];
                    if (fromRegisters) {
#pragma unroll
                        for (int i = 0; i < 4; ++i) x[i] = d[r][i];
                    } else if (virt) {
                        const int symA = sg.st[ch][(lane % G) + r * G], symB = sg.st[TABLES - 2 + ch][(lane % G) + r * G];
                        const int eA = 2 * (symA < S ? cc * 4 + symA : 4 * CP + cc);
                        const int eB = 2 * (symB < S ? cc * 4 + symB : 4 * CP + cc);
                        const double2 aLo = *reinterpret_cast<const double2*>(&sg.mat[ch][eA]);
                        const double2 aHi = *reinterpret_cast<const double2*>(&sg.mat[ch][10 * CP + eA]);
                        const double2 bLo = *reinterpret_cast<const double2*>(&sg.mat[TABLES - 2 + ch][eB]);
                        const double2 bHi = *reinterpret_cast<const double2*>(&sg.mat[TABLES - 2 + ch][10 * CP + eB]);
                        x[0] = aLo.x * bLo.x; x[1] = aLo.y * bLo.y; x[2] = aHi.x * bHi.x; x[3] = aHi.y * bHi.y;
                        roundCell<T>(x);
                    } else {
                        loadCell(xg + (size_t)r * G * 4, x);
                    }
#pragma unroll
                    for (int q = 0; q < 4; ++q)
                        u[q] = (Vi[4 * q] * x[0] + Vi[4 * q + 1] * x[1] + Vi[4 * q + 2] * x[2] + Vi[4 * q + 3] * x[3]) * e[q];
#pragma unroll
                    for (int i = 0; i < 4; ++i)
                        y[i] = absBits(A.V[4 * i] * u[0] + A.V[4 * i + 1] * u[1] + A.V[4 * i + 2] * u[2] + A.V[4 * i + 3] * u[3]);
#pragma unroll
                    for (int i = 0; i < 4; ++i) d[r][i] = ch == 0 ? y[i] : d[r][i] * y[i];
                }
            }
        }
        T* dg = static_cast<T*>(A.partials) + (size_t)cur.dest * A.stride + off0;
#pragma unroll
        for (int r = 0; r < R; ++r) {
            const int p = p0 + r * G;
            if (cur.sw >= 0) {
                double m = catValid ? fmax(fmax(d[r][0], d[r][1]), fmax(d[r][2], d[r][3])) : 0.0;
#pragma unroll
                for (int sh = G; sh < 32; sh <<= 1) m = fmax(m, __shfl_xor_sync(0xffffffffu, m, sh));
                if (m == 0.0) m = 1.0;
                const double inv = 1.0 / m;
#pragma unroll
                for (int i = 0; i < 4; ++i) d[r][i] *= inv;
                if (c == 0) A.scale[(size_t)cur.sw * A.Ppad + p] = A.logScalers ? log(m) : m;
            } else if (cur.sr >= 0) {
                double f = A.scale[(size_t)cur.sr * A.Ppad + p];
                if (A.logScalers) f = exp(f);
                const double inv = 1.0 / f;
#pragma unroll
                for (int i = 0; i < 4; ++i) d[r][i] *= inv;
            }
            roundCell<T>(d[r]);
            if (catValid) storeCell(dg + (size_t)r * G * 4, d[r]);
        }
        asm volatile("cp.async.wait_group 0;" ::: "memory");
        __syncwarp();
    }
}

template <int CP, int R, int MINB>
__global__ void __launch_bounds__(128, MINB)
k_walk4p(const WalkArgs A) {
    walk4pBody<double, CP, R, false>(A);
}

template <int CP, int R, int MINB>
__global__ void __launch_bounds__(128, MINB)
k_walk4ps(const WalkArgs A) {
    walk4pBody<float, CP, R, false>(A);
}

template <int CP, int R, int MINB>
__global__ void __launch_bounds__(128, MINB)
k_walk4pv(const WalkArgs A) {
    walk4pBody<double, CP, R, true>(A);
}

template <int CP, int R, int MINB>
__global__ void __launch_bounds__(128, MINB)
k_walk4pvs(const WalkArgs A) {
    walk4pBody<float, CP, R, true>(A);
}

template <typename T, int CP, int R, int MINB>
cudaError_t launchP(Instance* in, const WalkArgs& A, dim3 grid) {
    if constexpr (sizeof(T) == 4) k_walk4ps<CP, R, MINB><<<grid, 128, 0, in->stream>>>(A);
    else k_walk4p<CP, R, MINB><<<grid, 128, 0, in->stream>>>(A);
    return cudaGetLastError();
}

template <typename T, int CP, int R>
cudaError_t launchPV(Instance* in, const WalkArgs& A, dim3 grid) {
    if constexpr (sizeof(T) == 4) k_walk4pvs<CP, R, 3><<<grid, 128, 0, in->stream>>>(A);
    else k_walk4pv<CP, R, 3><<<grid, 128, 0, in->stream>>>(A);
    return cudaGetLastError();
}

__global__ void k_cherry_snapshot(const int4* items, const double* mats, size_t matStride, double* recipes, int blk) {
    const int4 it = items[blockIdx.x];
    for (int q = threadIdx.x; q < 2 * blk; q += blockDim.x)
        recipes[(size_t)it.x * 2 * blk + q] = mats[(size_t)(q < blk ? it.y : it.z) * matStride + q % blk];
}

template <typename T>
__device__ __forceinline__ void cherryStoreBody(const int4* items, int count, T* partials, size_t stride,
                                                const uint8_t* states, const double* recipes, int S, int C, int CP, int Ppad) {
    const int q = blockIdx.x * blockDim.x + threadIdx.x;
    if (q >= C * Ppad) return;
    const int c = q / Ppad, p = q - c * Ppad;
    for (int k = blockIdx.y; k < count; k += gridDim.y) {
        const int4 it = items[k];
        const int sA = states[(size_t)it.z * Ppad + p], sB = states[(size_t)it.w * Ppad + p];
        const double* ra = recipes + (size_t)it.y * 32 * CP;
        const double* rb = ra + 16 * CP;
        double v[4];
#pragma unroll
        for (int i = 0; i < 4; ++i) {
            const double a = sA < S ? ra[(sA * CP + c) * 4 + i] : (i < S ? 1.0 : 0.0);
            const double b = sB < S ? rb[(sB * CP + c) * 4 + i] : (i < S ? 1.0 : 0.0);
            v[i] = a * b;
        }
        roundCell<T>(v);
        storeCell(partials + (size_t)it.x * stride + (size_t)q * 4, v);
    }
}

__global__ void k_cherry_store(const int4* items, int count, double* partials, size_t stride, const uint8_t* states,
                               const double* recipes, int S, int C, int CP, int Ppad) {
    cherryStoreBody(items, count, partials, stride, states, recipes, S, C, CP, Ppad);
}

__global__ void k_cherry_store_f32(const int4* items, int count, float* partials, size_t stride, const uint8_t* states,
                                const double* recipes, int S, int C, int CP, int Ppad) {
    cherryStoreBody(items, count, partials, stride, states, recipes, S, C, CP, Ppad);
}

template <typename T, int CP, int R, bool ALIGNED, int MINB, int TIP>
cudaError_t launchK(Instance* in, const WalkArgs& A, dim3 grid) {
    if constexpr (sizeof(T) == 4) k_walk4es<CP, R, ALIGNED, MINB, TIP><<<grid, 128, 0, in->stream>>>(A);
    else k_walk4e<CP, R, ALIGNED, MINB, TIP><<<grid, 128, 0, in->stream>>>(A);
    return cudaGetLastError();
}

int phaseR(const Instance* in, int nSubs, int maxWindow) {
    const int G = 32 / in->matCP;
    const long walks = (long)nSubs * ((maxWindow + G * in->walkR - 1) / (G * in->walkR));
    if ((in->thinR1 && walks < (long)in->smCount * 8) || in->walkR == 1) return 1;
    if (in->matCP == 4 && (in->walkR == 8 || in->walkR == 2)) return in->walkR;
    return 4;
}

bool stagedWalk(const Instance* in, int R, bool aligned) {
    const int G = 32 / in->matCP;
    return aligned && in->Ppad % (G * R) == 0 && in->matCP <= 8 && G * R >= 4 && (R == 1 ? in->thinTipMode : in->tipMode) == 3;
}

template <typename T, int CP, int R>
cudaError_t launchR(Instance* in, WalkArgs& A, int nSubs, int maxWindow, bool aligned, bool virt) {
    constexpr int G = 32 / CP;
    constexpr int TIPD = CP <= 8 ? 2 : 0;
    const int warps = (maxWindow + G * R - 1) / (G * R);
    dim3 grid((warps + 3) / 4, nSubs);
    if constexpr (CP <= 8 && G * R >= 4) {
        if (stagedWalk(in, R, aligned)) {
            if (virt) {
                if constexpr (R == 8) return cudaErrorInvalidValue;
                else return launchPV<T, CP, R>(in, A, grid);
            }
            if constexpr (CP == 4) {
                const int minb = in->walkMinBlocksSet ? in->walkMinBlocks : 3;
                if (minb >= 6) return launchP<T, CP, R, 6>(in, A, grid);
                if (minb == 5) return launchP<T, CP, R, 5>(in, A, grid);
                if (minb == 3) return launchP<T, CP, R, 3>(in, A, grid);
            }
            return launchP<T, CP, R, 4>(in, A, grid);
        }
    }
    if (virt) return cudaErrorInvalidValue;
    if (!aligned || in->Ppad % (G * R) != 0) return launchK<T, CP, R, false, 4, TIPD>(in, A, grid);
    if constexpr (CP == 4 && R >= 2) {
        const int minb = in->walkMinBlocks, tip = in->tipMode;
        if (tip == 0) {
            if (minb >= 5) return launchK<T, CP, R, true, 5, 0>(in, A, grid);
            if (minb == 3) return launchK<T, CP, R, true, 3, 0>(in, A, grid);
            return launchK<T, CP, R, true, 4, 0>(in, A, grid);
        }
        if (tip == 1) {
            if (minb >= 5) return launchK<T, CP, R, true, 5, 1>(in, A, grid);
            return launchK<T, CP, R, true, 4, 1>(in, A, grid);
        }
        if (minb >= 6) return launchK<T, CP, R, true, 6, 2>(in, A, grid);
        if (minb == 5) return launchK<T, CP, R, true, 5, 2>(in, A, grid);
        if (minb == 3) return launchK<T, CP, R, true, 3, 2>(in, A, grid);
    }
    return launchK<T, CP, R, true, 4, TIPD>(in, A, grid);
}

template <typename T, int CP>
cudaError_t launchCP(Instance* in, WalkArgs& A, int nSubs, int maxWindow, bool aligned, bool virt) {
    const int R = phaseR(in, nSubs, maxWindow);
    if (R == 1) return launchR<T, CP, 1>(in, A, nSubs, maxWindow, aligned, virt);
    if constexpr (CP == 4) {
        if (R == 8) return launchR<T, CP, 8>(in, A, nSubs, maxWindow, aligned, virt);
        if (R == 2) return launchR<T, CP, 2>(in, A, nSubs, maxWindow, aligned, virt);
    }
    return launchR<T, CP, 4>(in, A, nSubs, maxWindow, aligned, virt);
}

}

bool walk4pServes(const Instance* in, int nSubs, int maxWindow) {
    if (in->matCP == 0) return false;
    const int R = phaseR(in, nSubs, maxWindow);
    return R != 8 && stagedWalk(in, R, true);
}

cudaError_t launchWalk4E(Instance* in, const Op4* dOps, const int4* dSubs, int nSubs, int maxWindow, bool aligned,
                         const double* eigen, const int4* dVirtTips) {
    const bool virt = dVirtTips != nullptr;
    if (nSubs <= 0) return cudaSuccess;
    WalkArgs A;
    A.ops = dOps; A.subs = dSubs; A.partials = in->partialsBase; A.stride = in->partialsElems;
    A.states = in->states8Base; A.mats = in->dMat; A.scale = in->dScale;
    A.S = in->S; A.C = in->C; A.Ppad = in->Ppad; A.logScalers = in->logScalers ? 1 : 0;
    A.matStride = in->matStride; A.matMmaOffset = 16 * in->matCP;
    A.evecs = in->dEvec;
    A.recipes = in->dRecipe;
    A.virtTips = dVirtTips;
    if (virt && in->dRecipe == nullptr) return cudaErrorInvalidValue;
    for (int q = 0; q < 16; ++q) { A.V[q] = eigen[q]; A.Vi[q] = eigen[16 + q]; }
    if (in->single) {
        switch (in->matCP) {
            case 1: return launchCP<float, 1>(in, A, nSubs, maxWindow, aligned, virt);
            case 2: return launchCP<float, 2>(in, A, nSubs, maxWindow, aligned, virt);
            case 8: return launchCP<float, 8>(in, A, nSubs, maxWindow, aligned, virt);
            default: return launchCP<float, 4>(in, A, nSubs, maxWindow, aligned, virt);
        }
    }
    switch (in->matCP) {
#ifndef B200_W4E_QUICK
        case 1: return launchCP<double, 1>(in, A, nSubs, maxWindow, aligned, virt);
        case 2: return launchCP<double, 2>(in, A, nSubs, maxWindow, aligned, virt);
        case 8: return launchCP<double, 8>(in, A, nSubs, maxWindow, aligned, virt);
        case 16: return launchCP<double, 16>(in, A, nSubs, maxWindow, aligned, virt);
        case 32: return launchCP<double, 32>(in, A, nSubs, maxWindow, aligned, virt);
#endif
        default: return launchCP<double, 4>(in, A, nSubs, maxWindow, aligned, virt);
    }
}

cudaError_t launchCherrySnapshot(Instance* in, const int4* dItems, int count) {
    if (count <= 0) return cudaSuccess;
    k_cherry_snapshot<<<count, 128, 0, in->stream>>>(dItems, in->dMat, in->matStride, in->dRecipe, 16 * in->matCP);
    return cudaGetLastError();
}

cudaError_t launchCherryStore(Instance* in, const int4* dItems, int count) {
    if (count <= 0) return cudaSuccess;
    const dim3 grid((in->C * in->Ppad + 255) / 256, std::min(count, 65535));
    if (in->single)
        k_cherry_store_f32<<<grid, 256, 0, in->stream>>>(dItems, count, reinterpret_cast<float*>(in->partialsBase),
                                                      in->partialsElems, in->states8Base, in->dRecipe, in->S, in->C,
                                                      in->matCP, in->Ppad);
    else
        k_cherry_store<<<grid, 256, 0, in->stream>>>(dItems, count, reinterpret_cast<double*>(in->partialsBase),
                                                     in->partialsElems, in->states8Base, in->dRecipe, in->S, in->C,
                                                     in->matCP, in->Ppad);
    return cudaGetLastError();
}

cudaError_t updateWalk4EGraph(cudaGraphExec_t exec, const std::vector<cudaGraphNode_t>& kernelNodes, const double* eigen) {
    for (cudaGraphNode_t node : kernelNodes) {
        cudaKernelNodeParams kp;
        cudaError_t e = cudaGraphKernelNodeGetParams(node, &kp);
        if (e != cudaSuccess) return e;
        if (kp.func == reinterpret_cast<void*>(k_cherry_snapshot)) continue;
        if (kp.kernelParams == nullptr || kp.kernelParams[0] == nullptr) return cudaErrorInvalidValue;
        WalkArgs A = *static_cast<const WalkArgs*>(kp.kernelParams[0]);
        for (int q = 0; q < 16; ++q) { A.V[q] = eigen[q]; A.Vi[q] = eigen[16 + q]; }
        void* args[1] = {&A};
        kp.kernelParams = args;
        kp.extra = nullptr;
        e = cudaGraphExecKernelNodeSetParams(exec, node, &kp);
        if (e != cudaSuccess) return e;
    }
    return cudaSuccess;
}

}
```

Measured before the change: 2359.

## Extend virtual cherries to three-tip clades computed on the fly in walk kernel

```diff
diff --git a/beast-mcmc_b200/csrc/api.cu b/beast-mcmc_b200/csrc/api.cu
--- a/beast-mcmc_b200/csrc/api.cu
+++ b/beast-mcmc_b200/csrc/api.cu
@@ -384,12 +384,13 @@
 
 cudaError_t launchPlan(Instance* in, const void* dOps, const void* dSubs, const std::vector<int>& phaseStart,
                        const std::vector<int>& phaseDepth, bool fourPath, int maxWindow, bool preOrder, int eigenSlot = -1,
-                       bool aligned = false, const void* dSnap = nullptr, int nSnap = 0, const void* dVirtTips = nullptr) {
+                       bool aligned = false, const void* dSnap = nullptr, int nSnap = 0, const void* dVirtTips = nullptr,
+                       bool clades = false) {
     const bool virt = dVirtTips != nullptr;
     cudaError_t e = cudaSuccess;
     if (nSnap > 0) {
         TimedScope ts(in, T_PARTIALS);
-        e = launchCherrySnapshot(in, static_cast<const int4*>(dSnap), nSnap);
+        e = launchCherrySnapshot(in, static_cast<const SnapItem*>(dSnap), nSnap);
     }
     for (size_t ph = 0; ph + 1 < phaseStart.size() && e == cudaSuccess; ++ph) {
         const int s0 = phaseStart[ph], s1 = phaseStart[ph + 1];
@@ -397,7 +398,8 @@
         TimedScope ts(in, T_PARTIALS);
         if (fourPath && eigenSlot >= 0 && !preOrder && (ph >= phaseDepth.size() || phaseDepth[ph] == 0)) {
             e = launchWalk4E(in, static_cast<const Op4*>(dOps), static_cast<const int4*>(dSubs) + s0, s1 - s0, maxWindow,
-                             aligned, in->hEigen.data() + (size_t)eigenSlot * 36, static_cast<const int4*>(dVirtTips));
+                             aligned, in->hEigen.data() + (size_t)eigenSlot * 36, static_cast<const int4*>(dVirtTips),
+                             clades);
             continue;
         }
         if (virt) return cudaErrorInvalidValue;
@@ -428,21 +430,21 @@
 
 cudaError_t storeCherries(Instance* in, const int* bufs, int count) {
     if (in->cherryTip1.empty()) return cudaSuccess;
-    std::vector<int4> items;
+    std::vector<StoreItem> items;
     for (int k = 0; k < count; ++k) {
         const int b = bufs[k];
         if (!validRange(b, in->nBuffers) || in->cherryTip1[b] < 0 || in->cherryStored[b]) continue;
-        items.push_back(make_int4(in->slotOf[b], b, in->cherryTip1[b], in->cherryTip2[b]));
+        items.push_back(StoreItem{in->slotOf[b], b, in->cherryTip1[b], in->cherryTip2[b], in->cherryTip3[b], 0, 0, 0});
         in->cherryStored[b] = 1;
     }
     if (items.empty()) return cudaSuccess;
-    const int4* dItems = static_cast<const int4*>(stage(in, items.data(), sizeof(int4) * items.size()));
+    const StoreItem* dItems = static_cast<const StoreItem*>(stage(in, items.data(), sizeof(StoreItem) * items.size()));
     cudaError_t e = cudaErrorMemoryAllocation;
     if (dItems != nullptr) {
         TimedScope ts(in, T_PARTIALS);
         e = launchCherryStore(in, dItems, (int)items.size());
     }
-    if (e != cudaSuccess) for (const int4& it : items) in->cherryStored[it.y] = 0;
+    if (e != cudaSuccess) for (const StoreItem& it : items) in->cherryStored[it.buf] = 0;
     return e;
 }
 
@@ -455,7 +457,8 @@
 cudaError_t settleCherriesOf(Instance* in, int t) {
     std::vector<int> deps;
     for (int b = 0; b < (int)in->cherryTip1.size(); ++b)
-        if (in->cherryTip1[b] >= 0 && (in->cherryTip1[b] == t || in->cherryTip2[b] == t)) deps.push_back(b);
+        if (in->cherryTip1[b] >= 0 && (in->cherryTip1[b] == t || in->cherryTip2[b] == t || in->cherryTip3[b] == t))
+            deps.push_back(b);
     const cudaError_t e = storeCherries(in, deps.data(), (int)deps.size());
     if (e == cudaSuccess) for (int b : deps) in->cherryTip1[b] = -1;
     return e;
@@ -465,7 +468,8 @@
     if (in->cherryTip1.empty()) return;
     for (const HostOp& o : hops) in->cherryTip1[o.dest] = -1;
     for (const CherryRef& c : cherries) {
-        in->cherryTip1[c.buf] = c.tip1; in->cherryTip2[c.buf] = c.tip2; in->cherryStored[c.buf] = 0;
+        in->cherryTip1[c.buf] = c.tip1; in->cherryTip2[c.buf] = c.tip2; in->cherryTip3[c.buf] = c.tip3;
+        in->cherryStored[c.buf] = 0;
     }
 }
 
@@ -519,9 +523,10 @@
                 memcmp(cp.key.data(), hops.data(), sizeof(HostOp) * (size_t)n) != 0)
                 continue;
             const int eigenSlot = cp.fourPath ? eigenFormSlot(in, hops) : -1;
-            bool stale = cp.readsVirtual && eigenSlot < 0;
+            bool stale = (cp.readsVirtual && eigenSlot < 0) || (cp.clades && cp.snapEigen != eigenSlot);
             for (const CherryRef& x : cp.external)
-                stale = stale || (x.tip1 >= 0 && (in->cherryTip1[x.buf] != x.tip1 || in->cherryTip2[x.buf] != x.tip2));
+                stale = stale || (x.tip1 >= 0 && (in->cherryTip1[x.buf] != x.tip1 || in->cherryTip2[x.buf] != x.tip2 ||
+                                                  in->cherryTip3[x.buf] != -1));
             if (stale) { cp.dropGraph(); cp.n = -1; continue; }
             CUDA_OK(storeExternal(in, cp.external));
             cp.lastUse = ++in->planClock;
@@ -548,7 +553,7 @@
                     cudaStreamBeginCapture(in->stream, cudaStreamCaptureModeThreadLocal) == cudaSuccess) {
                     const cudaError_t e1 = launchPlan(in, cp.dBlock, static_cast<char*>(cp.dBlock) + cp.subsOffset, cp.phaseStart,
                                                       cp.phaseDepth, cp.fourPath, cp.maxWindow, cp.preOrder, eigenSlot,
-                                                      !cp.byPartition, dSnap, nSnap, dTips);
+                                                      !cp.byPartition, dSnap, nSnap, dTips, cp.clades);
                     cp.graphEigen = eigenSlot;
                     cp.graphEigenGen = eigenGenNow;
                     cudaGraph_t g = nullptr;
@@ -589,7 +594,7 @@
             }
             CUDA_OK(launchPlan(in, cp.dBlock, static_cast<char*>(cp.dBlock) + cp.subsOffset, cp.phaseStart, cp.phaseDepth,
                                cp.fourPath, cp.maxWindow, cp.preOrder, eigenSlot, !cp.byPartition, dSnap, nSnap,
-                               dTips));
+                               dTips, cp.clades));
             CUDA_OK(accumulateInList(in, cp.cumGroups));
             noteScaleWrites(in, hops);
             noteCherryWrites(in, hops, cp.cherries);
@@ -607,9 +612,10 @@
     std::vector<int> firstWrite(in->nBuffers, n);
     for (int k = n - 1; k >= 0; --k) { written[hops[k].dest] = 1; firstWrite[hops[k].dest] = k; }
     std::vector<CherryRef> cherries;
-    std::vector<int4> snap;
+    std::vector<SnapItem> snap;
     std::vector<HostOp> kept;
     bool readsVirtual = false;
+    size_t nClades = 0;
     if (!in->cherryTip1.empty() && !byPartition && !preOrder && eigenSlot >= 0 && !in->stackTail) {
         std::vector<int> writes(in->nBuffers, 0), firstRead(in->nBuffers, n);
         for (int k = 0; k < n; ++k) {
@@ -617,21 +623,53 @@
             firstRead[hops[k].c1] = std::min(firstRead[hops[k].c1], k);
             firstRead[hops[k].c2] = std::min(firstRead[hops[k].c2], k);
         }
+        std::vector<int> cherryOf(in->nBuffers, -1);
+        auto plain = [&](const HostOp& o, int k) {
+            return o.sw == BEAGLE_OP_NONE && o.sr == BEAGLE_OP_NONE && o.cum == BEAGLE_OP_NONE && writes[o.dest] == 1 &&
+                   firstRead[o.dest] > k;
+        };
+        std::vector<char> virt(n, 0);
         for (int k = 0; k < n; ++k) {
             const HostOp& o = hops[k];
-            if (in->states8[o.c1] != nullptr && in->states8[o.c2] != nullptr && o.sw == BEAGLE_OP_NONE &&
-                o.sr == BEAGLE_OP_NONE && o.cum == BEAGLE_OP_NONE && writes[o.dest] == 1 && firstRead[o.dest] > k) {
-                cherries.push_back(CherryRef{o.dest, o.c1, o.c2});
-                snap.push_back(make_int4(o.dest, o.m1, o.m2, 0));
-            } else {
-                kept.push_back(o);
-            }
-        }
-        if (kept.empty()) { cherries.clear(); snap.clear(); }
+            if (in->states8[o.c1] != nullptr && in->states8[o.c2] != nullptr && plain(o, k)) {
+                virt[k] = 1;
+                cherryOf[o.dest] = (int)cherries.size();
+                cherries.push_back(CherryRef{o.dest, o.c1, o.c2, -1});
+                snap.push_back(SnapItem{o.dest, o.m1, o.m2, -1, -1, eigenSlot, 0, 0});
+            }
+        }
+        std::vector<int> cladeOp(in->nBuffers, -1);
+        const bool clades = in->virtualCherries >= 2 && walk4pcServes(in);
+        for (int k = 0; k < n && clades; ++k) {
+            const HostOp& o = hops[k];
+            if (virt[k] || !plain(o, k)) continue;
+            const bool tip1 = in->states8[o.c1] != nullptr, tip2 = in->states8[o.c2] != nullptr;
+            if (tip1 != tip2 && cherryOf[tip1 ? o.c2 : o.c1] >= 0) { virt[k] = 2; cladeOp[o.dest] = k; }
+        }
+        for (int k = 0; k < n && clades; ++k)
+            if (!virt[k] && cladeOp[hops[k].c1] >= 0 && cladeOp[hops[k].c2] >= 0 && hops[k].c1 != hops[k].c2) {
+                virt[cladeOp[hops[k].c2]] = 0;
+                cladeOp[hops[k].c2] = -1;
+            }
+        for (int k = 0; k < n; ++k) {
+            if (virt[k] != 2) continue;
+            const HostOp& o = hops[k];
+            const bool tip1 = in->states8[o.c1] != nullptr;
+            const int x = tip1 ? o.c2 : o.c1, t = tip1 ? o.c1 : o.c2;
+            const CherryRef ch = cherries[cherryOf[x]];
+            const SnapItem cs = snap[cherryOf[x]];
+            cherries.push_back(CherryRef{o.dest, ch.tip1, ch.tip2, t});
+            snap.push_back(SnapItem{o.dest, cs.m1, cs.m2, tip1 ? o.m1 : o.m2, tip1 ? o.m2 : o.m1, eigenSlot, 0, 0});
+            ++nClades;
+        }
+        for (int k = 0; k < n; ++k)
+            if (!virt[k]) kept.push_back(hops[k]);
+        if (kept.empty()) { cherries.clear(); snap.clear(); nClades = 0; }
         readsVirtual = !cherries.empty();
         for (const HostOp& o : hops)
             for (int c : {o.c1, o.c2})
-                readsVirtual = readsVirtual || (!written[c] && in->states32[c] == nullptr && in->cherryTip1[c] >= 0);
+                readsVirtual = readsVirtual || (!written[c] && in->states32[c] == nullptr && in->cherryTip1[c] >= 0 &&
+                                                in->cherryTip3[c] < 0);
     }
     Plan plan;
     int maxWindow = in->Ppad;
@@ -653,7 +691,7 @@
         if (!served) {
             readsVirtual = false;
             if (!cherries.empty()) {
-                cherries.clear(); snap.clear(); kept.clear();
+                cherries.clear(); snap.clear(); kept.clear(); nClades = 0;
                 planPhases(hops, in->nBuffers, in->reorder != 0, in->phaseT, wantSubsFor(in->Ppad), in->phaseTmin,
                            in->phaseSmall, plan);
             }
@@ -662,8 +700,9 @@
     }
     const std::vector<HostOp>& L = cherries.empty() ? hops : kept;
     const int nL = (int)L.size();
-    std::vector<int> vt1(readsVirtual ? in->nBuffers : 0, -1), vt2(readsVirtual ? in->nBuffers : 0, -1);
-    for (const CherryRef& c : cherries) { vt1[c.buf] = c.tip1; vt2[c.buf] = c.tip2; }
+    std::vector<int> vt1(readsVirtual ? in->nBuffers : 0, -1), vt2(readsVirtual ? in->nBuffers : 0, -1),
+        vt3(readsVirtual ? in->nBuffers : 0, -1);
+    for (const CherryRef& c : cherries) { vt1[c.buf] = c.tip1; vt2[c.buf] = c.tip2; vt3[c.buf] = c.tip3; }
     std::vector<CherryRef> external;
     {
         std::vector<char> seen(in->nBuffers, 0);
@@ -671,8 +710,8 @@
             for (int c : {hops[k].c1, hops[k].c2}) {
                 if (firstWrite[c] < k || in->states32[c] != nullptr || seen[c]) continue;
                 seen[c] = 1;
-                const bool virt = readsVirtual && !written[c] && in->cherryTip1[c] >= 0;
-                external.push_back(CherryRef{c, virt ? in->cherryTip1[c] : -1, virt ? in->cherryTip2[c] : -1});
+                const bool virt = readsVirtual && !written[c] && in->cherryTip1[c] >= 0 && in->cherryTip3[c] < 0;
+                external.push_back(CherryRef{c, virt ? in->cherryTip1[c] : -1, virt ? in->cherryTip2[c] : -1, -1});
                 if (virt) { vt1[c] = in->cherryTip1[c]; vt2[c] = in->cherryTip2[c]; }
             }
     }
@@ -771,7 +810,8 @@
     std::vector<CumGroup> cumGroups;
     std::vector<DevOp> dops(fourPath ? 0 : nL);
     std::vector<Op4> ops4(fourPath ? nL : 0);
-    std::vector<int4> virtTips(readsVirtual ? nL : 0);
+    const int tipsPerOp = nClades > 0 ? 2 : 1;
+    std::vector<int4> virtTips(readsVirtual ? tipsPerOp * nL : 0);
     for (int pos = 0; pos < nL; ++pos) {
         const HostOp& o = L[order[pos]];
         const bool t1 = in->states32[o.c1] != nullptr;
@@ -814,24 +854,33 @@
         const int cum = -1;
         if (fourPath) {
             Op4& d = ops4[pos];
-            const bool v1 = readsVirtual && !t1 && vt1[o.c1] >= 0, v2 = readsVirtual && !t2 && vt1[o.c2] >= 0;
+            bool v1 = readsVirtual && !t1 && vt1[o.c1] >= 0, v2 = readsVirtual && !t2 && vt1[o.c2] >= 0;
+            bool k1 = v1 && vt3[o.c1] >= 0, k2 = v2 && vt3[o.c2] >= 0;
+            int c1 = o.c1, c2 = o.c2, m1 = o.m1, m2 = o.m2;
+            bool s1 = t1, s2 = t2;
+            if (k2) { std::swap(c1, c2); std::swap(m1, m2); std::swap(s1, s2); std::swap(v1, v2); std::swap(k1, k2); }
             d.dest = in->slotOf[o.dest];
-            d.c1 = t1 ? -(o.c1 + 1) : v1 ? o.c1 : in->slotOf[o.c1];
-            d.c2 = t2 ? -(o.c2 + 1) : v2 ? o.c2 : in->slotOf[o.c2];
-            d.m1 = o.m1; d.m2 = o.m2; d.sw = o.sw; d.sr = o.sr; d.cum = cum;
+            d.c1 = s1 ? -(c1 + 1) : v1 ? c1 : in->slotOf[c1];
+            d.c2 = s2 ? -(c2 + 1) : v2 ? c2 : in->slotOf[c2];
+            d.m1 = m1; d.m2 = m2; d.sw = o.sw; d.sr = o.sr; d.cum = cum;
             d.pBegin = pBegin; d.pEnd = pEnd;
             d.slots = (unsigned)(srcSlot1 & 0xFF) | ((unsigned)(srcSlot2 & 0xFF) << 8) | ((unsigned)(dstSlot & 0xFF) << 16);
-            d.pad_ = o.kind | (v1 ? 4 : 0) | (v2 ? 8 : 0);
+            d.pad_ = o.kind | (v1 ? 4 : 0) | (v2 ? 8 : 0) | (k1 ? 16 : 0);
             d.pfA = d.pfB = 0; d.pfM1 = d.pfM2 = -1;
-            if (readsVirtual)
-                virtTips[pos] = make_int4(v1 ? vt1[o.c1] : 0, v1 ? vt2[o.c1] : 0, v2 ? vt1[o.c2] : 0, v2 ? vt2[o.c2] : 0);
-            if (in->forward && !(maxDepth > 0 && subStack[subOfPos[pos]]) && pos > plan.subs[subOfPos[pos]].begin) {
+            if (readsVirtual && tipsPerOp == 1) {
+                virtTips[pos] = make_int4(v1 ? vt1[c1] : 0, v1 ? vt2[c1] : 0, v2 ? vt1[c2] : 0, v2 ? vt2[c2] : 0);
+            } else if (readsVirtual) {
+                virtTips[2 * pos] = v1 ? make_int4(vt1[c1], vt2[c1], vt3[c1], 0) : make_int4(0, 0, -1, 0);
+                virtTips[2 * pos + 1] = v2 ? make_int4(vt1[c2], vt2[c2], -1, 0) : make_int4(0, 0, -1, 0);
+            }
+            if (in->forward && !k1 && !(maxDepth > 0 && subStack[subOfPos[pos]]) && pos > plan.subs[subOfPos[pos]].begin) {
                 const Op4& pv = ops4[pos - 1];
                 if (pv.pBegin == d.pBegin && pv.pEnd == d.pEnd) {
-                    if (!t1 && !v1 && d.c1 == pv.dest) d.pad_ |= 2;
-                    else if (!preOrder && !t2 && !v2 && d.c2 == pv.dest) {
+                    if (!s1 && !v1 && d.c1 == pv.dest) d.pad_ |= 2;
+                    else if (!preOrder && !s2 && !v2 && d.c2 == pv.dest) {
                         std::swap(d.c1, d.c2); std::swap(d.m1, d.m2);
-                        if (readsVirtual) { int4& t = virtTips[pos]; t = make_int4(t.z, t.w, t.x, t.y); }
+                        if (readsVirtual && tipsPerOp == 1) { int4& t = virtTips[pos]; t = make_int4(t.z, t.w, t.x, t.y); }
+                        else if (readsVirtual) std::swap(virtTips[2 * pos], virtTips[2 * pos + 1]);
                         d.pad_ = (d.pad_ & ~12) | (v1 ? 8 : 0) | 2;
                     }
                 }
@@ -890,12 +939,13 @@
     if (fourPath && getenv("B200_BEAGLE_DEBUG")) {
         int fwd = 0, internal = 0;
         for (const Op4& d : ops4) { fwd += (d.pad_ & 2) != 0; internal += (d.c1 >= 0) + (d.c2 >= 0); }
-        fprintf(stderr, "[b200-beagle] plan: %d ops (%zu virtual cherries), %zu subtrees, %d phases, %d internal children, "
-                "%d forwarded in registers\n", nL, cherries.size(), plan.subs.size(), nPhases, internal, fwd);
+        fprintf(stderr, "[b200-beagle] plan: %d ops (%zu virtual cherries) (%zu virtual clades), %zu subtrees, %d phases, "
+                "%d internal children, %d forwarded in registers\n", nL, cherries.size() - nClades, nClades, plan.subs.size(),
+                nPhases, internal, fwd);
     }
     const size_t opBytes = (fourPath ? sizeof(Op4) : sizeof(DevOp)) * (size_t)nL;
     const size_t subBytes = sizeof(Sub) * plan.subs.size();
-    const size_t snapBytes = sizeof(int4) * snap.size();
+    const size_t snapBytes = sizeof(SnapItem) * snap.size();
     const size_t subsOffset = (opBytes + 255) & ~size_t(255);
     const size_t snapOffset = subsOffset + ((subBytes + 255) & ~size_t(255));
     const size_t tipsBytes = sizeof(int4) * virtTips.size();
@@ -920,7 +970,7 @@
     for (size_t ph = 0; ph + 1 < plan.phaseStart.size(); ++ph) depths[ph] = (maxDepth > 0 && ph < phaseDepth.size()) ? phaseDepth[ph] : 0;
     cudaError_t e = launchPlan(in, dOps, dSubs, plan.phaseStart, depths, fourPath, maxWindow, preOrder, eigenSlot, !byPartition,
                                static_cast<char*>(dOps) + snapOffset, (int)snap.size(),
-                               readsVirtual ? static_cast<char*>(dOps) + tipsOffset : nullptr);
+                               readsVirtual ? static_cast<char*>(dOps) + tipsOffset : nullptr, nClades > 0);
     if (e == cudaSuccess) e = accumulateInList(in, cumGroups);
     noteScaleWrites(in, hops);
     if (e == cudaSuccess) noteCherryWrites(in, hops, cherries);
@@ -945,6 +995,7 @@
             slot->key = hops; slot->n = n; slot->byPartition = byPartition; slot->epoch = in->bufferEpoch;
             slot->subsOffset = subsOffset; slot->snapOffset = snapOffset; slot->tipsOffset = tipsOffset;
             slot->cherries = cherries; slot->external = external; slot->readsVirtual = readsVirtual;
+            slot->snapEigen = eigenSlot; slot->clades = nClades > 0;
             slot->phaseStart = plan.phaseStart; slot->phaseDepth = depths;
             slot->fourPath = fourPath; slot->maxWindow = maxWindow; slot->preOrder = preOrder;
             slot->lastUse = ++in->planClock;
@@ -1087,7 +1138,7 @@
     in->eigenWalk = envInt("B200_EIGEN_WALK", 1);
     in->tipMode = envInt("B200_TIP_MODE", 3);
     in->thinTipMode = envInt("B200_THIN_TIP_MODE", in->tipMode);
-    in->virtualCherries = envInt("B200_VIRTUAL_CHERRIES", 1);
+    in->virtualCherries = envInt("B200_VIRTUAL_CHERRIES", 2);
     in->walkBlock = 128;
     in->walkVariant = envInt("B200_WALK_VARIANT", 0);
     in->reorder = envInt("B200_REORDER", 1);
@@ -1137,9 +1188,10 @@
     alloc(&in->dMat, matElems);
     if (in->matCP > 0) alloc(&in->dEvec, (size_t)in->nMatrices * in->matCP * 4);
     if (in->matCP > 0 && in->matCP <= 8 && in->virtualCherries) {
-        alloc(&in->dRecipe, (size_t)in->nBuffers * 32 * in->matCP);
+        alloc(&in->dRecipe, (size_t)in->nBuffers * recipeRow(in->matCP));
         in->cherryTip1.assign(in->nBuffers, -1);
         in->cherryTip2.assign(in->nBuffers, -1);
+        in->cherryTip3.assign(in->nBuffers, -1);
         in->cherryStored.assign(in->nBuffers, 0);
     }
     if (in->matCP > 0 && in->matCP <= 8) {
diff --git a/beast-mcmc_b200/csrc/engine.h b/beast-mcmc_b200/csrc/engine.h
--- a/beast-mcmc_b200/csrc/engine.h
+++ b/beast-mcmc_b200/csrc/engine.h
@@ -32,7 +32,10 @@
     int pfA, pfB, pfM1, pfM2;
 };
 
-struct CherryRef { int buf, tip1, tip2; };
+struct CherryRef { int buf, tip1, tip2, tip3; };
+__host__ __device__ constexpr int recipeRow(int cp) { return 52 * cp + 32; }
+struct alignas(16) SnapItem { int buf, m1, m2, m3, mx, eigen, pad0, pad1; };
+struct alignas(16) StoreItem { int slot, buf, tip1, tip2, tip3, pad0, pad1, pad2; };
 
 template <typename T> struct EdgeRefT { const T* post; const int* states; const T* pre; const double* D; double len; };
 using EdgeRef = EdgeRefT<double>;
@@ -49,6 +52,8 @@
     size_t capacity = 0, subsOffset = 0, snapOffset = 0, tipsOffset = 0;
     std::vector<CherryRef> cherries, external;
     bool readsVirtual = false;
+    bool clades = false;
+    int snapEigen = -1;
     std::vector<int> phaseStart, phaseDepth;
     int maxWindow = 0;
     long lastUse = 0;
@@ -129,8 +134,8 @@
     int eigenWalk = 1;
     int tipMode = 2;
     int thinTipMode = 3;
-    int virtualCherries = 1;
-    std::vector<int> cherryTip1, cherryTip2;
+    int virtualCherries = 2;
+    std::vector<int> cherryTip1, cherryTip2, cherryTip3;
     std::vector<char> cherryStored;
     double* dRecipe = nullptr;
     double* dRates = nullptr;
@@ -218,10 +223,11 @@
 cudaError_t launchWalk4(Instance* in, const Op4* dOps, const int4* dSubs, int nSubs, int stackDepth, int maxWindow, bool preOrder);
 cudaError_t updateWalk4EGraph(cudaGraphExec_t exec, const std::vector<cudaGraphNode_t>& kernelNodes, const double* eigen);
 cudaError_t launchWalk4E(Instance* in, const Op4* dOps, const int4* dSubs, int nSubs, int maxWindow, bool aligned,
-                         const double* eigen, const int4* dVirtTips);
+                         const double* eigen, const int4* dVirtTips, bool clades);
 bool walk4pServes(const Instance* in, int nSubs, int maxWindow);
-cudaError_t launchCherrySnapshot(Instance* in, const int4* dItems, int count);
-cudaError_t launchCherryStore(Instance* in, const int4* dItems, int count);
+bool walk4pcServes(const Instance* in);
+cudaError_t launchCherrySnapshot(Instance* in, const SnapItem* dItems, int count);
+cudaError_t launchCherryStore(Instance* in, const StoreItem* dItems, int count);
 cudaError_t launchWalkGeneric(Instance* in, const DevOp* dOps, const int4* dSubs, int nSubs, int maxWindow, bool preOrder);
 size_t edgeDerivativeWorkspace(const Instance* in, int count);
 cudaError_t launchEdgeDerivatives(Instance* in, const EdgeRefT<void>* dEdges, int count, const double* weights, double* outPerPattern,
diff --git a/beast-mcmc_b200/csrc/walk4e.cu b/beast-mcmc_b200/csrc/walk4e.cu
--- a/beast-mcmc_b200/csrc/walk4e.cu
+++ b/beast-mcmc_b200/csrc/walk4e.cu
@@ -1,12 +1,25 @@
 #include "engine.h"
 #include "walk4.cuh"
 
+#include <type_traits>
+
 namespace b200 {
 
 namespace {
 
 __device__ __forceinline__ double absBits(double v) {
     return __hiloint2double(__double2hiint(v) & 0x7fffffff, __double2loint(v));
+}
+
+__device__ __forceinline__ void eigenBranch(const double (&Vi)[16], const double* V, const double (&e)[4],
+                                            const double (&x)[4], double (&y)[4]) {
+    double u[4];
+#pragma unroll
+    for (int k = 0; k < 4; ++k)
+        u[k] = (Vi[4 * k] * x[0] + Vi[4 * k + 1] * x[1] + Vi[4 * k + 2] * x[2] + Vi[4 * k + 3] * x[3]) * e[k];
+#pragma unroll
+    for (int i = 0; i < 4; ++i)
+        y[i] = absBits(V[4 * i] * u[0] + V[4 * i + 1] * u[1] + V[4 * i + 2] * u[2] + V[4 * i + 3] * u[3]);
 }
 
 template <typename T, int CP, int R, bool ALIGNED, bool FIRST, int TIP>
@@ -76,7 +89,7 @@
     for (int r = 0; r < R; ++r) {
         const int p = p0 + r * G;
         const bool live = ALIGNED || (catValid && p >= pBegin && p < pEnd);
-        double x[4], u[4], y[4];
+        double x[4], y[4];
         int s = 0;
         if (tip) {
             s = live ? (int)__ldg(t + p) : S;
@@ -90,12 +103,7 @@
         } else {
             x[0] = x[1] = x[2] = x[3] = 0.0;
         }
-#pragma unroll
-        for (int k = 0; k < 4; ++k)
-            u[k] = (Vi[4 * k] * x[0] + Vi[4 * k + 1] * x[1] + Vi[4 * k + 2] * x[2] + Vi[4 * k + 3] * x[3]) * e[k];
-#pragma unroll
-        for (int i = 0; i < 4; ++i)
-            y[i] = absBits(A.V[4 * i] * u[0] + A.V[4 * i + 1] * u[1] + A.V[4 * i + 2] * u[2] + A.V[4 * i + 3] * u[3]);
+        eigenBranch(Vi, A.V, e, x, y);
         if (tip && s >= S) {
 #pragma unroll
             for (int i = 0; i < 4; ++i) y[i] = (i < S) ? 1.0 : 0.0;
@@ -207,24 +215,31 @@
     asm volatile("cp.async.ca.shared.global [%0], [%1], %2;" :: "r"(sAddr), "l"(gmemSrc), "n"(BYTES) : "memory");
 }
 
-template <int CP, int R, bool VIRT>
+template <int CP, int R, int VIRT>
 struct WarpStage {
-    static constexpr int G = 32 / CP, NP = G * R, TABLES = VIRT ? 4 : 2;
+    static constexpr int G = 32 / CP, NP = G * R, TABLES = VIRT == 2 ? 5 : VIRT ? 4 : 2;
     double mat[TABLES][5 * CP * 4];
-    double ev[2][CP * 4];
+    double ev[VIRT == 2 ? 3 : 2][CP * 4];
     alignas(16) unsigned char st[TABLES][NP < 16 ? 16 : NP];
 };
 
-template <typename T, int CP, int R, bool VIRT>
+template <int CP, int R, int VIRT>
+constexpr bool kDynamicStages = sizeof(WarpStage<CP, R, VIRT>) * 8 + 2048 > 48 * 1024;
+
+template <typename T, int CP, int R, int VIRT>
 __device__ __forceinline__ void walk4pBody(const WalkArgs& A) {
     constexpr int G = 32 / CP, NP = G * R;
     constexpr int PIECE = NP < 16 ? NP : 16;
     static_assert(NP % PIECE == 0 && (PIECE == 4 || PIECE == 8 || PIECE == 16), "state-byte staging");
     constexpr int TABLES = WarpStage<CP, R, VIRT>::TABLES;
-    constexpr int RECQ = sizeof(Op4) / 16 + (VIRT ? 1 : 0);
-    __shared__ __align__(16) WarpStage<CP, R, VIRT> stages[4][2];
+    constexpr int TIPQ = VIRT == 2 ? 2 : VIRT ? 1 : 0;
+    constexpr int RECQ = sizeof(Op4) / 16 + TIPQ;
+    constexpr int T2 = VIRT ? 2 : 0, T3 = VIRT == 2 ? 4 : 0;
+    using StaticStage = std::conditional_t<kDynamicStages<CP, R, VIRT>, char, WarpStage<CP, R, VIRT>>;
+    __shared__ __align__(16) StaticStage stages[4][2];
+    extern __shared__ __align__(16) unsigned char stageSmem[];
     __shared__ __align__(16) Op4 rings[4][4];
-    __shared__ __align__(16) int4 tipRings[4][VIRT ? 4 : 1];
+    __shared__ __align__(16) int4 tipRings[4][TIPQ ? 4 * TIPQ : 1];
     int lane;
     asm volatile("mov.u32 %0, %%laneid;" : "=r"(lane));
     const int wib = threadIdx.x >> 5;
@@ -238,7 +253,9 @@
     const int cc = catValid ? c : 0;
     const size_t off0 = ((size_t)cc * A.Ppad + p0) * 4;
     const int last = range.y - 1, S = A.S;
-    WarpStage<CP, R, VIRT>* stage = stages[wib];
+    WarpStage<CP, R, VIRT>* stage;
+    if constexpr (kDynamicStages<CP, R, VIRT>) stage = reinterpret_cast<WarpStage<CP, R, VIRT>*>(stageSmem) + 2 * wib;
+    else stage = stages[wib];
     Op4* ring = rings[wib];
     int4* tipRing = tipRings[wib];
 
@@ -252,7 +269,8 @@
             cpAsync16(&tab[(q & 1) * 10 * CP + 2 * (((q >> 1) % CP) * 4 + q / (2 * CP))], src + 2 * q);
     };
     auto fetchRecord = [&](int j) {
-        if (VIRT && lane == RECQ - 1) cpAsync16(&tipRing[j & 3], A.virtTips + j);
+        if (VIRT == 1 && lane == RECQ - 1) cpAsync16(&tipRing[j & 3], A.virtTips + j);
+        else if (VIRT == 2 && lane >= RECQ - 2) cpAsync16(&tipRing[2 * (j & 3) + lane - (RECQ - 2)], A.virtTips + 2 * (size_t)j + lane - (RECQ - 2));
         else cpAsync16(reinterpret_cast<char*>(&ring[j & 3]) + 16 * lane, reinterpret_cast<const char*>(A.ops + j) + 16 * lane);
     };
     struct Rec { int dest, c1, c2, sw, sr, flags, pfA, pfB; };
@@ -271,21 +289,29 @@
                 stageBlock(sg.mat[ch], A.mats + (size_t)m * A.matStride);
             } else {
                 if (virt) {
-                    const double* rcp = A.recipes + (size_t)child * 32 * CP;
+                    const double* rcp = A.recipes + (size_t)child * recipeRow(CP);
                     stageBlock(sg.mat[ch], rcp);
-                    stageBlock(sg.mat[TABLES - 2 + ch], rcp + 16 * CP);
+                    stageBlock(sg.mat[T2 + ch], rcp + 16 * CP);
+                    if (VIRT == 2 && ch == 0 && (flags & 16)) {
+                        stageBlock(sg.mat[T3], rcp + 32 * CP);
+                        if (lane < CP * 2) cpAsync16(&sg.ev[T2][2 * lane], rcp + 48 * CP + 2 * lane);
+                    }
                 }
                 if (lane < CP * 2) cpAsync16(&sg.ev[ch][2 * lane], A.evecs + (size_t)m * CP * 4 + 2 * lane);
             }
         }
         constexpr int SL = NP / PIECE;
+        static_assert(RECQ + TABLES * SL <= 64, "record and state-byte pieces: two instructions at most");
         auto statePiece = [&](int q) {
             const int t = q / SL, piece = q % SL, ch = t & 1;
             const int child = ch == 0 ? rec.y : rec.z;
             int tip = t < 2 && child < 0 ? -child - 1 : -1;
-            if (VIRT && (flags & (4 << ch)) != 0) {
+            if (VIRT == 1 && (flags & (4 << ch)) != 0) {
                 const int4 vt = tipRing[j & 3];
                 tip = t == 0 ? vt.x : t == 1 ? vt.z : t == 2 ? vt.y : vt.w;
+            } else if (VIRT == 2 && (flags & (4 << ch)) != 0) {
+                const int4 vt = tipRing[2 * (j & 3) + ch];
+                tip = t < 2 ? vt.x : t < 4 ? vt.y : vt.z;
             }
             if (tip >= 0) cpAsyncSmall<PIECE>(&sg.st[t][PIECE * piece], A.states + (size_t)tip * A.Ppad + pBase + PIECE * piece);
         };
@@ -340,6 +366,39 @@
                     if (ch == 0) { d[r][0] = lo.x; d[r][1] = lo.y; d[r][2] = hi.x; d[r][3] = hi.y; }
                     else { d[r][0] *= lo.x; d[r][1] *= lo.y; d[r][2] *= hi.x; d[r][3] *= hi.y; }
                 }
+            } else if (VIRT == 2 && ch == 0 && (cur.flags & 16) != 0) {
+                const double2* ep = reinterpret_cast<const double2*>(&sg.ev[0][cc * 4]);
+                const double2 e01 = ep[0], e23 = ep[1];
+                const double e[4] = {e01.x, e01.y, e23.x, e23.y};
+                double Vr[16];
+#pragma unroll
+                for (int q = 0; q < 16; ++q) asm volatile("mov.f64 %0, %1;" : "=d"(Vr[q]) : "d"(A.V[q]));
+#pragma unroll
+                for (int r = 0; r < R; ++r) {
+                    double x[4], y[4];
+                    const int symA = sg.st[0][(lane % G) + r * G], symB = sg.st[T2][(lane % G) + r * G];
+                    const int eA = 2 * (symA < S ? cc * 4 + symA : 4 * CP + cc);
+                    const int eB = 2 * (symB < S ? cc * 4 + symB : 4 * CP + cc);
+                    const double2 aLo = *reinterpret_cast<const double2*>(&sg.mat[0][eA]);
+                    const double2 aHi = *reinterpret_cast<const double2*>(&sg.mat[0][10 * CP + eA]);
+                    const double2 bLo = *reinterpret_cast<const double2*>(&sg.mat[T2][eB]);
+                    const double2 bHi = *reinterpret_cast<const double2*>(&sg.mat[T2][10 * CP + eB]);
+                    x[0] = aLo.x * bLo.x; x[1] = aLo.y * bLo.y; x[2] = aHi.x * bHi.x; x[3] = aHi.y * bHi.y;
+                    roundCell<T>(x);
+                    const double2* xp = reinterpret_cast<const double2*>(&sg.ev[T2][cc * 4]);
+                    const double2 x01 = xp[0], x23 = xp[1];
+                    const double ex[4] = {x01.x, x01.y, x23.x, x23.y};
+                    eigenBranch(Vi, Vr, ex, x, y);
+                    const int symC = sg.st[T3][(lane % G) + r * G];
+                    const int eC = 2 * (symC < S ? cc * 4 + symC : 4 * CP + cc);
+                    const double2 cLo = *reinterpret_cast<const double2*>(&sg.mat[T3][eC]);
+                    const double2 cHi = *reinterpret_cast<const double2*>(&sg.mat[T3][10 * CP + eC]);
+                    x[0] = y[0] * cLo.x; x[1] = y[1] * cLo.y; x[2] = y[2] * cHi.x; x[3] = y[3] * cHi.y;
+                    roundCell<T>(x);
+                    eigenBranch(Vi, Vr, e, x, y);
+#pragma unroll
+                    for (int i = 0; i < 4; ++i) d[r][i] = y[i];
+                }
             } else {
                 const double2* ep = reinterpret_cast<const double2*>(&sg.ev[ch][cc * 4]);
                 const double2 e01 = ep[0], e23 = ep[1];
@@ -349,29 +408,24 @@
                 const T* xg = static_cast<const T*>(A.partials) + (size_t)child * A.stride + off0;
 #pragma unroll
                 for (int r = 0; r < R; ++r) {
-                    double x[4], u[4], y[4];
+                    double x[4], y[4];
                     if (fromRegisters) {
 #pragma unroll
                         for (int i = 0; i < 4; ++i) x[i] = d[r][i];
                     } else if (virt) {
-                        const int symA = sg.st[ch][(lane % G) + r * G], symB = sg.st[TABLES - 2 + ch][(lane % G) + r * G];
+                        const int symA = sg.st[ch][(lane % G) + r * G], symB = sg.st[T2 + ch][(lane % G) + r * G];
                         const int eA = 2 * (symA < S ? cc * 4 + symA : 4 * CP + cc);
                         const int eB = 2 * (symB < S ? cc * 4 + symB : 4 * CP + cc);
                         const double2 aLo = *reinterpret_cast<const double2*>(&sg.mat[ch][eA]);
                         const double2 aHi = *reinterpret_cast<const double2*>(&sg.mat[ch][10 * CP + eA]);
-                        const double2 bLo = *reinterpret_cast<const double2*>(&sg.mat[TABLES - 2 + ch][eB]);
-                        const double2 bHi = *reinterpret_cast<const double2*>(&sg.mat[TABLES - 2 + ch][10 * CP + eB]);
+                        const double2 bLo = *reinterpret_cast<const double2*>(&sg.mat[T2 + ch][eB]);
+                        const double2 bHi = *reinterpret_cast<const double2*>(&sg.mat[T2 + ch][10 * CP + eB]);
                         x[0] = aLo.x * bLo.x; x[1] = aLo.y * bLo.y; x[2] = aHi.x * bHi.x; x[3] = aHi.y * bHi.y;
                         roundCell<T>(x);
                     } else {
                         loadCell(xg + (size_t)r * G * 4, x);
                     }
-#pragma unroll
-                    for (int q = 0; q < 4; ++q)
-                        u[q] = (Vi[4 * q] * x[0] + Vi[4 * q + 1] * x[1] + Vi[4 * q + 2] * x[2] + Vi[4 * q + 3] * x[3]) * e[q];
-#pragma unroll
-                    for (int i = 0; i < 4; ++i)
-                        y[i] = absBits(A.V[4 * i] * u[0] + A.V[4 * i + 1] * u[1] + A.V[4 * i + 2] * u[2] + A.V[4 * i + 3] * u[3]);
+                    eigenBranch(Vi, A.V, e, x, y);
 #pragma unroll
                     for (int i = 0; i < 4; ++i) d[r][i] = ch == 0 ? y[i] : d[r][i] * y[i];
                 }
@@ -408,25 +462,37 @@
 template <int CP, int R, int MINB>
 __global__ void __launch_bounds__(128, MINB)
 k_walk4p(const WalkArgs A) {
-    walk4pBody<double, CP, R, false>(A);
+    walk4pBody<double, CP, R, 0>(A);
 }
 
 template <int CP, int R, int MINB>
 __global__ void __launch_bounds__(128, MINB)
 k_walk4ps(const WalkArgs A) {
-    walk4pBody<float, CP, R, false>(A);
+    walk4pBody<float, CP, R, 0>(A);
 }
 
 template <int CP, int R, int MINB>
 __global__ void __launch_bounds__(128, MINB)
 k_walk4pv(const WalkArgs A) {
-    walk4pBody<double, CP, R, true>(A);
+    walk4pBody<double, CP, R, 1>(A);
 }
 
 template <int CP, int R, int MINB>
 __global__ void __launch_bounds__(128, MINB)
 k_walk4pvs(const WalkArgs A) {
-    walk4pBody<float, CP, R, true>(A);
+    walk4pBody<float, CP, R, 1>(A);
+}
+
+template <int CP, int R, int MINB>
+__global__ void __launch_bounds__(128, MINB)
+k_walk4pc(const WalkArgs A) {
+    walk4pBody<double, CP, R, 2>(A);
+}
+
+template <int CP, int R, int MINB>
+__global__ void __launch_bounds__(128, MINB)
+k_walk4pcs(const WalkArgs A) {
+    walk4pBody<float, CP, R, 2>(A);
 }
 
 template <typename T, int CP, int R, int MINB>
@@ -437,28 +503,57 @@
 }
 
 template <typename T, int CP, int R>
-cudaError_t launchPV(Instance* in, const WalkArgs& A, dim3 grid) {
-    if constexpr (sizeof(T) == 4) k_walk4pvs<CP, R, 3><<<grid, 128, 0, in->stream>>>(A);
-    else k_walk4pv<CP, R, 3><<<grid, 128, 0, in->stream>>>(A);
+cudaError_t launchPV(Instance* in, const WalkArgs& A, dim3 grid, int level) {
+    if (level == 1) {
+        if constexpr (sizeof(T) == 4) k_walk4pvs<CP, R, 3><<<grid, 128, 0, in->stream>>>(A);
+        else k_walk4pv<CP, R, 3><<<grid, 128, 0, in->stream>>>(A);
+        return cudaGetLastError();
+    }
+    auto kernel = sizeof(T) == 4 ? k_walk4pcs<CP, R, 3> : k_walk4pc<CP, R, 3>;
+    size_t smem = 0;
+    if constexpr (kDynamicStages<CP, R, 2>) {
+        smem = sizeof(WarpStage<CP, R, 2>) * 8;
+        const cudaError_t e = cudaFuncSetAttribute(kernel, cudaFuncAttributeMaxDynamicSharedMemorySize, (int)smem);
+        if (e != cudaSuccess) return e;
+    }
+    kernel<<<grid, 128, smem, in->stream>>>(A);
     return cudaGetLastError();
 }
 
-__global__ void k_cherry_snapshot(const int4* items, const double* mats, size_t matStride, double* recipes, int blk) {
-    const int4 it = items[blockIdx.x];
-    for (int q = threadIdx.x; q < 2 * blk; q += blockDim.x)
-        recipes[(size_t)it.x * 2 * blk + q] = mats[(size_t)(q < blk ? it.y : it.z) * matStride + q % blk];
+__global__ void k_cherry_snapshot(const SnapItem* items, const double* mats, size_t matStride, const double* evecs,
+                                  const double* eigen, int S, double* recipes, int CP) {
+    const SnapItem it = items[blockIdx.x];
+    const int blk = 16 * CP;
+    double* row = recipes + (size_t)it.buf * recipeRow(CP);
+    const int blocks = it.m3 >= 0 ? 3 : 2;
+    for (int q = threadIdx.x; q < blocks * blk; q += blockDim.x) {
+        const int b = q / blk;
+        row[q] = mats[(size_t)(b == 0 ? it.m1 : b == 1 ? it.m2 : it.m3) * matStride + q % blk];
+    }
+    if (it.m3 < 0) return;
+    for (int q = threadIdx.x; q < 4 * CP + 32; q += blockDim.x) {
+        double v;
+        if (q < 4 * CP) {
+            v = evecs[(size_t)it.mx * CP * 4 + q];
+        } else {
+            const int r = q - 4 * CP, i = (r >> 2) & 3, k = r & 3;
+            const double* E = eigen + (size_t)it.eigen * (2 * S * S + 2 * S) + (r >> 4) * S * S;
+            v = (i < S && k < S) ? E[i * S + k] : 0.0;
+        }
+        row[3 * blk + q] = v;
+    }
 }
 
 template <typename T>
-__device__ __forceinline__ void cherryStoreBody(const int4* items, int count, T* partials, size_t stride,
+__device__ __forceinline__ void cherryStoreBody(const StoreItem* items, int count, T* partials, size_t stride,
                                                 const uint8_t* states, const double* recipes, int S, int C, int CP, int Ppad) {
     const int q = blockIdx.x * blockDim.x + threadIdx.x;
     if (q >= C * Ppad) return;
     const int c = q / Ppad, p = q - c * Ppad;
     for (int k = blockIdx.y; k < count; k += gridDim.y) {
-        const int4 it = items[k];
-        const int sA = states[(size_t)it.z * Ppad + p], sB = states[(size_t)it.w * Ppad + p];
-        const double* ra = recipes + (size_t)it.y * 32 * CP;
+        const StoreItem it = items[k];
+        const int sA = states[(size_t)it.tip1 * Ppad + p], sB = states[(size_t)it.tip2 * Ppad + p];
+        const double* ra = recipes + (size_t)it.buf * recipeRow(CP);
         const double* rb = ra + 16 * CP;
         double v[4];
 #pragma unroll
@@ -468,16 +563,30 @@
             v[i] = a * b;
         }
         roundCell<T>(v);
-        storeCell(partials + (size_t)it.x * stride + (size_t)q * 4, v);
-    }
-}
-
-__global__ void k_cherry_store(const int4* items, int count, double* partials, size_t stride, const uint8_t* states,
+        if (it.tip3 >= 0) {
+            const double* rc = ra + 32 * CP;
+            const double* V = ra + 52 * CP;
+            double Vi[16], e[4], y[4];
+#pragma unroll
+            for (int j = 0; j < 16; ++j) Vi[j] = V[16 + j];
+#pragma unroll
+            for (int j = 0; j < 4; ++j) e[j] = ra[48 * CP + c * 4 + j];
+            eigenBranch(Vi, V, e, v, y);
+            const int sC = states[(size_t)it.tip3 * Ppad + p];
+#pragma unroll
+            for (int i = 0; i < 4; ++i) v[i] = y[i] * (sC < S ? rc[(sC * CP + c) * 4 + i] : (i < S ? 1.0 : 0.0));
+            roundCell<T>(v);
+        }
+        storeCell(partials + (size_t)it.slot * stride + (size_t)q * 4, v);
+    }
+}
+
+__global__ void k_cherry_store(const StoreItem* items, int count, double* partials, size_t stride, const uint8_t* states,
                                const double* recipes, int S, int C, int CP, int Ppad) {
     cherryStoreBody(items, count, partials, stride, states, recipes, S, C, CP, Ppad);
 }
 
-__global__ void k_cherry_store_f32(const int4* items, int count, float* partials, size_t stride, const uint8_t* states,
+__global__ void k_cherry_store_f32(const StoreItem* items, int count, float* partials, size_t stride, const uint8_t* states,
                                 const double* recipes, int S, int C, int CP, int Ppad) {
     cherryStoreBody(items, count, partials, stride, states, recipes, S, C, CP, Ppad);
 }
@@ -503,7 +612,7 @@
 }
 
 template <typename T, int CP, int R>
-cudaError_t launchR(Instance* in, WalkArgs& A, int nSubs, int maxWindow, bool aligned, bool virt) {
+cudaError_t launchR(Instance* in, WalkArgs& A, int nSubs, int maxWindow, bool aligned, int virt) {
     constexpr int G = 32 / CP;
     constexpr int TIPD = CP <= 8 ? 2 : 0;
     const int warps = (maxWindow + G * R - 1) / (G * R);
@@ -512,7 +621,7 @@
         if (stagedWalk(in, R, aligned)) {
             if (virt) {
                 if constexpr (R == 8) return cudaErrorInvalidValue;
-                else return launchPV<T, CP, R>(in, A, grid);
+                else return launchPV<T, CP, R>(in, A, grid, virt);
             }
             if constexpr (CP == 4) {
                 const int minb = in->walkMinBlocksSet ? in->walkMinBlocks : 3;
@@ -544,7 +653,7 @@
 }
 
 template <typename T, int CP>
-cudaError_t launchCP(Instance* in, WalkArgs& A, int nSubs, int maxWindow, bool aligned, bool virt) {
+cudaError_t launchCP(Instance* in, WalkArgs& A, int nSubs, int maxWindow, bool aligned, int virt) {
     const int R = phaseR(in, nSubs, maxWindow);
     if (R == 1) return launchR<T, CP, 1>(in, A, nSubs, maxWindow, aligned, virt);
     if constexpr (CP == 4) {
@@ -556,6 +665,10 @@
 
 }
 
+bool walk4pcServes(const Instance* in) {
+    return in->matCP == 2 || in->matCP == 4 || (in->matCP == 8 && !in->single);
+}
+
 bool walk4pServes(const Instance* in, int nSubs, int maxWindow) {
     if (in->matCP == 0) return false;
     const int R = phaseR(in, nSubs, maxWindow);
@@ -563,8 +676,8 @@
 }
 
 cudaError_t launchWalk4E(Instance* in, const Op4* dOps, const int4* dSubs, int nSubs, int maxWindow, bool aligned,
-                         const double* eigen, const int4* dVirtTips) {
-    const bool virt = dVirtTips != nullptr;
+                         const double* eigen, const int4* dVirtTips, bool clades) {
+    const int virt = dVirtTips == nullptr ? 0 : clades ? 2 : 1;
     if (nSubs <= 0) return cudaSuccess;
     WalkArgs A;
     A.ops = dOps; A.subs = dSubs; A.partials = in->partialsBase; A.stride = in->partialsElems;
@@ -596,13 +709,14 @@
     }
 }
 
-cudaError_t launchCherrySnapshot(Instance* in, const int4* dItems, int count) {
+cudaError_t launchCherrySnapshot(Instance* in, const SnapItem* dItems, int count) {
     if (count <= 0) return cudaSuccess;
-    k_cherry_snapshot<<<count, 128, 0, in->stream>>>(dItems, in->dMat, in->matStride, in->dRecipe, 16 * in->matCP);
+    k_cherry_snapshot<<<count, 128, 0, in->stream>>>(dItems, in->dMat, in->matStride, in->dEvec, in->dEigen, in->S,
+                                                     in->dRecipe, in->matCP);
     return cudaGetLastError();
 }
 
-cudaError_t launchCherryStore(Instance* in, const int4* dItems, int count) {
+cudaError_t launchCherryStore(Instance* in, const StoreItem* dItems, int count) {
     if (count <= 0) return cudaSuccess;
     const dim3 grid((in->C * in->Ppad + 255) / 256, std::min(count, 65535));
     if (in->single)
```

After: 2587 (median of 6 runs). +9.6%, better.
